# zsc/MOSS-TTSD

Measured on AMD Instinct MI355X. Metric: audio codec tokens/sec/node (decode, bf16, batch 32 @ 4k ctx), higher is better.
Workload: dtype bf16; 1 GPU; configs[2]: batch 32 synthetic dialogues/GPU, 4k-token KV context, top-k/top-p sampling on 8 channels, decode steps at full context; batch_per_gpu=32, context=4096, prompt=512, layers=28, hidden=2048, parallelism=dp1 (batch shard, no per-step collective)

## Files before the change

### include/mtts.h

```cpp
#ifndef MTTS_H
#define MTTS_H

#include <stdint.h>

#ifdef __cplusplus
extern "C" {
#endif

#define MTTS_OK 0
#define MTTS_EINVAL (-1)
#define MTTS_EHIP (-2)
#define MTTS_ENOMEM (-3)
#define MTTS_ESTATE (-4)

#define MTTS_CHANNELS 8

typedef struct MttsConfig {
    int32_t vocab_size;
    int32_t hidden_size;
    int32_t intermediate_size;
    int32_t num_hidden_layers;
    int32_t num_attention_heads;
    int32_t num_key_value_heads;
    int32_t head_dim;
    int32_t channels;
    int32_t speech_vocab_size;
    int32_t speech_pad_token;
    int32_t speech_range_lo;
    int32_t speech_range_hi;
    int32_t eos_token_id;
    int32_t max_position;
    float rms_norm_eps;
    int32_t max_batch;
    int32_t max_seq_len;
    int32_t kv_pool_pages;
    int32_t dtype;
} MttsConfig;
#define MTTS_DTYPE_BF16 0
#define MTTS_DTYPE_F32 1
#define MTTS_DTYPE_F16 2

typedef struct MttsSamplerCfg {
    int32_t do_sample;
    int32_t top_k;
    float top_p;
    float one_minus_top_p;
    float temperature;
    float repetition_penalty;
} MttsSamplerCfg;

typedef struct MttsEngine MttsEngine;

const char* mtts_last_error(void);
int32_t mtts_version(void);

int32_t mtts_engine_create(const MttsConfig* cfg, int32_t device, MttsEngine** out);
int32_t mtts_engine_destroy(MttsEngine* e);

int32_t mtts_bind_weight(MttsEngine* e, const char* name, const void* dev_bf16,
                         int64_t rows, int64_t cols, void* stream);
int32_t mtts_bind_rope(MttsEngine* e, const void* dev_cos_bf16, const void* dev_sin_bf16,
                       int32_t rows, void* stream);
int32_t mtts_weights_ready(MttsEngine* e);

int32_t mtts_generate(MttsEngine* e, const int64_t* host_input_ids, const uint8_t* host_attention_mask,
                      int32_t B, int32_t T, int32_t max_length,
                      const MttsSamplerCfg* sampler, uint64_t seed,
                      int64_t* host_out_ids, int32_t out_capacity, int32_t* out_len,
                      const int64_t* host_forced, int32_t forced_len, int64_t* host_decisions,
                      void* stream);

int32_t mtts_begin(MttsEngine* e, const int64_t* host_input_ids, const uint8_t* host_attention_mask,
                   int32_t B, int32_t T, int32_t max_length,
                   const MttsSamplerCfg* sampler, uint64_t seed, void* stream);
int32_t mtts_step(MttsEngine* e, int32_t n_steps, void* stream);
int32_t mtts_sync_state(MttsEngine* e, int32_t* steps_done, int32_t* all_finished, void* stream);
int32_t mtts_read_generated(MttsEngine* e, int64_t* host_gen, int32_t capacity_steps, int32_t* n_steps);
int32_t mtts_set_output_scores(MttsEngine* e, int32_t on);
int32_t mtts_read_scores(MttsEngine* e, float* host_lp, int32_t capacity_steps, int32_t* n_steps);
int32_t mtts_slot_read_scores(MttsEngine* e, int32_t slot, float* host_rows, int32_t capacity_steps, int32_t* n_steps);
int32_t mtts_score(MttsEngine* e, const int64_t* host_input_ids, const uint8_t* host_attention_mask,
                   const int64_t* host_labels, int32_t B, int32_t T, float* host_logp, void* stream);
int32_t mtts_read_logits(MttsEngine* e, uint16_t* host_logits0, uint16_t* host_logits17, void* stream);
int32_t mtts_read_logits_f32(MttsEngine* e, float* host_logits0, float* host_logits17, void* stream);
int32_t mtts_sched_open(MttsEngine* e, int32_t B, int32_t gen_cap, const MttsSamplerCfg* sampler, void* stream);
int32_t mtts_slot_submit(MttsEngine* e, int32_t slot, const int64_t* host_ids, int32_t T, int32_t max_length, uint64_t seed,
                         void* stream);
int32_t mtts_slot_submit_row(MttsEngine* e, int32_t slot, const int64_t* host_ids, int32_t T, int32_t max_length, uint64_t seed,
                             int32_t row_id, void* stream);
int32_t mtts_set_row_ids(MttsEngine* e, const int32_t* host_row_ids, int32_t n);
int32_t mtts_set_takes(MttsEngine* e, int32_t n);
int32_t mtts_slot_fork(MttsEngine* e, int32_t src_slot, int32_t dst_slot, uint64_t seed, int32_t row_id, void* stream);
int32_t mtts_slot_states(MttsEngine* e, int32_t* host_state, void* stream);
int32_t mtts_slot_read(MttsEngine* e, int32_t slot, int64_t* host_rows, int32_t capacity_steps, int32_t* n_steps);
int32_t mtts_read_seq_state(MttsEngine* e, int32_t* host_nas, int32_t* host_unfinished, int32_t* host_kv_len, void* stream);
int32_t mtts_slot_evict(MttsEngine* e, int32_t slot, void* stream);
int32_t mtts_kv_pool_state(MttsEngine* e, int32_t* total_pages, int32_t* free_pages, int32_t* max_pages_per_seq);
int32_t mtts_read_page_table(MttsEngine* e, int32_t* host_table, int32_t* host_n_pages);
int32_t mtts_set_forced_mode(MttsEngine* e, int32_t as_draw);
int32_t mtts_debug_read_device_page_table(MttsEngine* e, int32_t* host_table, void* stream);
int32_t mtts_export_codes(MttsEngine* e, int32_t first, int32_t n, int64_t* dev_codes, void* stream);
int32_t mtts_profile_enable(MttsEngine* e, int32_t on);
int32_t mtts_profile_read(MttsEngine* e, int32_t which, double* total_ms, int64_t* launches, int64_t* bytes);

int32_t mtts_debug_set_kv_len(MttsEngine* e, int32_t kv_len);
int32_t mtts_debug_kv_pack_stats(MttsEngine* e, int64_t* out6);
int32_t mtts_k_attn_bench(MttsEngine* e, int32_t phase, int32_t iters, float* avg_ms, int64_t* bytes_per_launch);
int32_t mtts_k_gemm_bench(int32_t N, int32_t K, int32_t epi, int32_t ksplit, int32_t waves, int32_t copies,
                          int32_t iters, float* avg_us);

int32_t mtts_k_gemm_bf16(const void* dev_w, const void* dev_x, void* dev_y,
                         int32_t M, int32_t N, int32_t K, int32_t ksplit, void* stream);
int64_t mtts_debug_gemm_depth_launches(void);
int64_t mtts_debug_attn_row_launches(void);
int32_t mtts_k_attn_section(const float* dev_slabs, int32_t ksplit, const void* dev_qnw, const void* dev_knw, const void* dev_cos,
                            const void* dev_sin, float eps, const void* dev_k, const void* dev_v, const int32_t* host_lens,
                            const int32_t* host_page_table, int32_t R, int32_t Lmax, int32_t nq, int32_t nkv, int32_t sealed,
                            int32_t path, void* dev_out, void* dev_kcache, void* dev_vcache, void* dev_kpack, void* dev_vpack,
                            void* stream);
int32_t mtts_k_gemm_swiglu_bf16(const void* dev_w, const void* dev_x, void* dev_y,
                                int32_t M, int32_t N, int32_t K, void* stream);
int32_t mtts_k_rmsnorm(const void* dev_x, const void* dev_w, void* dev_y,
                       int32_t rows, int32_t n, float eps, void* stream);
int32_t mtts_k_rope_kvwrite(const void* dev_qkv, const int32_t* host_pos, const void* dev_qnorm, const void* dev_knorm,
                            const void* dev_cos, const void* dev_sin, int32_t R, int32_t nq, int32_t nkv, float eps,
                            void* dev_q, void* dev_k, void* dev_v, void* stream);
int32_t mtts_k_paged_attn_decode(const void* dev_q, const void* dev_k, const void* dev_v, const int32_t* host_lens,
                                 const int32_t* host_page_table, int32_t R, int32_t Lmax, int32_t nq, int32_t nkv,
                                 void* dev_out, void* stream);
int32_t mtts_k_kv_seal(const void* dev_pages, int32_t npages, void* dev_sealed, int32_t as_k, void* stream);
int32_t mtts_k_head_ce(const void* dev_w, const void* dev_x, const int32_t* host_labels, int32_t M, int32_t N, int32_t K,
                       int32_t n_valid, int32_t segments, float* dev_logp, void* stream);
int32_t mtts_k_sample(const void* dev_logits_bf16, int32_t rows, int32_t vocab,
                      const void* dev_history_bitmap, const MttsSamplerCfg* cfg,
                      int32_t mask_id, uint64_t seed, int32_t step, int32_t channel,
                      int32_t* dev_tokens, void* stream);
int32_t mtts_k_sample_scores(const void* dev_logits_bf16, int32_t rows, int32_t vocab,
                             const void* dev_history_bitmap, const MttsSamplerCfg* cfg,
                             int32_t mask_id, uint64_t seed, int32_t step, int32_t channel,
                             int32_t* dev_tokens, float* dev_logp, void* stream);

typedef struct MttsCodecConfig {
    int32_t nq, codebook_size, rvq_dim, quant_out_dim;
    int32_t adapter_layers, adapter_dim, adapter_heads, adapter_ffn, adapter_max_pos;
    int32_t up_stride;
    int32_t dec_layers, dec_dim, dec_heads, dec_ffn, dec_max_pos, mel_bins;
    int32_t voc_dim, voc_inter, voc_layers, n_fft, hop;
    int32_t mel_n_fft, mel_hop, mel_frames;
    int32_t enc_layers, enc_dim, enc_heads, enc_ffn, enc_max_pos;
    int32_t sem_adapter_layers, pre_rvq_layers, down_pool;
} MttsCodecConfig;

typedef struct MttsCodec MttsCodec;
const char* mtts_codec_last_error(void);
int32_t mtts_codec_create(const MttsCodecConfig* cfg, int32_t device, MttsCodec** out);
int32_t mtts_codec_destroy(MttsCodec* c);
int32_t mtts_codec_bind(MttsCodec* c, const char* role, const float* dev_f32, int64_t n, void* stream);
int32_t mtts_codec_detokenize(MttsCodec* c, const int64_t* dev_codes, const int32_t* host_lens, int32_t B, int32_t T,
                              float* dev_wav, void* stream);
int32_t mtts_codec_detokenize_async(MttsCodec* c, const int64_t* dev_codes, const int32_t* host_lens, int32_t B, int32_t T,
                                    float* dev_wav, void* stream);
int32_t mtts_codec_check(MttsCodec* c, void* stream);
int32_t mtts_codec_tokenize(MttsCodec* c, const float* dev_wav, const int32_t* host_lens, int32_t B, int32_t nsamp,
                            int64_t* dev_codes, int32_t* host_code_lens, void* stream);
int32_t mtts_k_gemm_f32(const float* dev_a, const float* dev_w, const float* dev_bias, float* dev_c,
                        int32_t M, int32_t N, int32_t K, int32_t act, void* stream);
int32_t mtts_k_gemm_planes_bench(int32_t M, int32_t N, int32_t K, int32_t flags, int32_t tile_code, int32_t iters,
                                 float* avg_us, int32_t* code_used);

#ifdef __cplusplus
}
#endif
#endif
```

### moss-ttsd_amd/csrc/attn.hip

```cpp
#include "launch.h"
#include <algorithm>
#include <atomic>
#include <cstdlib>
#ifndef MTTS_PK_WAVES
#define MTTS_PK_WAVES 0
#endif
#if MTTS_PK_WAVES
#define PK_OCC(PK) __attribute__((amdgpu_waves_per_eu((PK) ? MTTS_PK_WAVES : 1, (PK) ? MTTS_PK_WAVES : 8)))
#else
#define PK_OCC(PK)
#endif

__device__ __forceinline__ uint32_t u4c(const u32x4_t& v, int c) { return c == 0 ? v.x : c == 1 ? v.y : c == 2 ? v.z : v.w; }
__device__ __forceinline__ void pk_unit(const u32x4_t* pk, int j, uint32_t w[4]) {
    const uint32_t L0 = u4c(pk[j >> 1], 2 * (j & 1)), L1 = u4c(pk[j >> 1], 2 * (j & 1) + 1);
    const uint32_t N = u4c(pk[8 + (j >> 2)], j & 3);
    const uint32_t lo = pk[12].x, hi = pk[12].y;
    const uint32_t HA = ((N & 0x08080808u) << 4) | __builtin_amdgcn_perm(hi, lo, N & 0x07070707u);
    const uint32_t HB = (N & 0x80808080u) | __builtin_amdgcn_perm(hi, lo, (N >> 4) & 0x07070707u);
    w[0] = __builtin_amdgcn_perm(HA, L0, 0x05010400u);
    w[1] = __builtin_amdgcn_perm(HA, L0, 0x07030602u);
    w[2] = __builtin_amdgcn_perm(HB, L1, 0x05010400u);
    w[3] = __builtin_amdgcn_perm(HB, L1, 0x07030602u);
}

__host__ __device__ constexpr int pk_order(int i) { return i == 0 ? 12 : (i - 1) % 3 == 0 ? 8 + (i - 1) / 3 : 2 * ((i - 1) / 3) + (i - 1) % 3 - 1; }
__device__ bool seal_encode(const u32x4_t (&v)[16], u32x4_t* __restrict__ pk, uint32_t spare, bool unfit) {
    unsigned long long b0 = 0ull, b1 = 0ull;
#pragma unroll
    for (int j = 0; j < 16; ++j)
#pragma unroll
        for (int c = 0; c < 4; ++c)
#pragma unroll
            for (int h = 0; h < 2; ++h) {
                const uint32_t e = (u4c(v[j], c) >> (8 + 16 * h)) & 0x7fu;
                if (e & 64u) b1 |= 1ull << (e & 63u);
                else b0 |= 1ull << e;
            }
    const int n0 = __popcll(b0), n = n0 + __popcll(b1);
    if (n > 8 || unfit) {
        pk[12 * 64] = u32x4_t{0u, 0u, spare, 1u};
        return false;
    }
    unsigned long long dict = 0ull;
    {
        unsigned long long t0 = b0, t1 = b1;
        for (int i = 0; i < n; ++i) {
            uint32_t e;
            if (t0) { e = __ffsll((long long)t0) - 1; t0 &= t0 - 1; }
            else { e = 64 + __ffsll((long long)t1) - 1; t1 &= t1 - 1; }
            dict |= (unsigned long long)e << (8 * i);
        }
    }
    auto code = [&](uint32_t half) -> uint32_t {
        const uint32_t e = (half >> 8) & 0x7fu;
        const uint32_t rank = (e & 64u) ? n0 + __popcll(b1 & ((1ull << (e & 63u)) - 1ull)) : __popcll(b0 & ((1ull << e) - 1ull));
        return ((half >> 12) & 8u) | rank;
    };
    uint32_t lowp[32], nib[16];
#pragma unroll
    for (int j = 0; j < 16; ++j) {
        uint32_t N = 0u;
#pragma unroll
        for (int g = 0; g < 2; ++g) {
            uint32_t L = 0u;
#pragma unroll
            for (int k = 0; k < 4; ++k) {
                const uint32_t half = (u4c(v[j], 2 * g + (k >> 1)) >> (16 * (k & 1))) & 0xffffu;
                L |= (half & 0xffu) << (8 * k);
                N |= code(half) << (8 * k + 4 * g);
            }
            lowp[2 * j + g] = L;
        }
        nib[j] = N;
    }
#pragma unroll
    for (int u = 0; u < 8; ++u) pk[u * 64] = u32x4_t{lowp[4 * u], lowp[4 * u + 1], lowp[4 * u + 2], lowp[4 * u + 3]};
#pragma unroll
    for (int u = 0; u < 4; ++u) pk[(8 + u) * 64] = u32x4_t{nib[4 * u], nib[4 * u + 1], nib[4 * u + 2], nib[4 * u + 3]};
    pk[12 * 64] = u32x4_t{(uint32_t)dict, (uint32_t)(dict >> 32), spare, 0u};
    return true;
}
__device__ bool seal_lane(const u32x4_t* __restrict__ raw, u32x4_t* __restrict__ pk) {
    u32x4_t v[16];
#pragma unroll
    for (int j = 0; j < 16; ++j) v[j] = raw[j * 64];
    return seal_encode(v, pk, 0u, false);
}
__device__ bool seal_lane_k(const u32x4_t* __restrict__ raw, u32x4_t* __restrict__ pk, uint8_t* __restrict__ lds, int lane) {
    u32x4_t v[16];
#pragma unroll
    for (int j = 0; j < 16; ++j) v[j] = raw[j * 64];
    __builtin_amdgcn_wave_barrier();
    uint32_t* row = (uint32_t*)(lds + lane * 128);
#pragma unroll
    for (int j = 0; j < 16; ++j)
#pragma unroll
        for (int c = 0; c < 4; c += 2) {
            const uint32_t a = u4c(v[j], c), b = u4c(v[j], c + 1);
            row[2 * j + (c >> 1)] = ((a >> 7) & 0xffu) | (((a >> 23) & 0xffu) << 8) | (((b >> 7) & 0xffu) << 16) | (((b >> 23) & 0xffu) << 24);
        }
    __builtin_amdgcn_wave_barrier();
    uint32_t a0 = 0u, a1 = 0u, n0 = 0u, n1 = 0u;
    for (int t = 0; t < 64; ++t) {
        const uint32_t e = *(const uint16_t*)(lds + t * 128 + 2 * lane);
        a0 += e & 0xffu; n0 += (e & 0xffu) ? 1u : 0u;
        a1 += e >> 8; n1 += (e >> 8) ? 1u : 0u;
    }
    const int s0 = n0 ? min(max((int)((a0 + n0 / 2) / n0) - 125, -127), 127) : 0;
    const int s1 = n1 ? min(max((int)((a1 + n1 / 2) / n1) - 125, -127), 127) : 0;
    int8_t* sv = (int8_t*)(lds + 8192);
    sv[2 * lane] = (int8_t)s0;
    sv[2 * lane + 1] = (int8_t)s1;
    __builtin_amdgcn_wave_barrier();
    bool unfit = false;
#pragma unroll
    for (int j = 0; j < 16; ++j) {
        uint32_t w[4] = {v[j].x, v[j].y, v[j].z, v[j].w};
#pragma unroll
        for (int c = 0; c < 4; ++c) {
            const uint32_t sh = *(const uint16_t*)(sv + 8 * j + 2 * c);
            uint32_t out = 0u;
#pragma unroll
            for (int h = 0; h < 2; ++h) {
                uint32_t b = (w[c] >> (16 * h)) & 0xffffu;
                const int sft = (int)(int8_t)((sh >> (8 * h)) & 0xffu);
                const int e = (int)((b >> 7) & 0xffu);
                if (e == 0) {
                    if ((b & 0x7fu) && sft) unfit = true;
                } else {
                    const int e2 = e - sft;
                    if (e == 255 ? sft != 0 : (e2 < 1 || e2 > 254)) unfit = true;
                    else b = (b - ((uint32_t)sft << 7)) & 0xffffu;
                }
                out |= b << (16 * h);
            }
            w[c] = out;
        }
        v[j] = u32x4_t{w[0], w[1], w[2], w[3]};
    }
    return seal_encode(v, pk, ((uint32_t)s0 & 0xffu) | (((uint32_t)s1 & 0xffu) << 8), unfit);
}
__device__ bool seal_lane_v(const u32x4_t* __restrict__ raw, u32x4_t* __restrict__ pk, uint8_t* __restrict__ lds, int lane) {
    u32x4_t v[16];
#pragma unroll
    for (int j = 0; j < 16; ++j) v[j] = raw[j * 64];
    const int sub = lane >> 5;
    __builtin_amdgcn_wave_barrier();
    uint32_t* row = (uint32_t*)(lds + lane * 128);
#pragma unroll
    for (int it = 0; it < 16; ++it)
#pragma unroll
        for (int h = 0; h < 2; ++h) {
            uint32_t sum = 0u, cnt = 0u;
#pragma unroll
            for (int c = 0; c < 4; ++c) {
                const uint32_t e = (u4c(v[it], c) >> (7 + 16 * h)) & 0xffu;
                sum += e;
                cnt += e ? 1u : 0u;
            }
            row[2 * it + h] = sum | (cnt << 16);
        }
    __builtin_amdgcn_wave_barrier();
    int mean;
    {
        const int t = lane, st = (t >> 1) & 1, j = 2 * (t >> 2) + (t & 1);
        uint32_t tot = 0u, cn = 0u;
        for (int d = 0; d < 32; ++d) {
            const uint32_t w = ((const uint32_t*)(lds + (st * 32 + d) * 128))[j];
            tot += w & 0xffffu;
            cn += w >> 16;
// ... 1214 lines not shown
```

### moss-ttsd_amd/csrc/engine.h

```cpp
#pragma once
#include <hip/hip_runtime.h>

#include <algorithm>
#include <cstdarg>
#include <cstdio>
#include <cstdlib>
#include <cstring>
#include <memory>
#include <string>
#include <vector>

#include "launch.h"

#define MTTS_LOCAL __attribute__((visibility("hidden")))
extern MTTS_LOCAL thread_local char g_err[512];
MTTS_LOCAL int fail(int code, const char* fmt, ...) __attribute__((format(printf, 2, 3)));
#define HIPCHK(x)                                                                          \
    do {                                                                                   \
        hipError_t _e = (x);                                                               \
        if (_e != hipSuccess) return fail(MTTS_EHIP, "%s: %s (%s:%d)", #x, hipGetErrorString(_e), __FILE__, __LINE__); \
    } while (0)
#define TRY(x)             \
    do {                   \
        int _r = (x);      \
        if (_r) return _r; \
    } while (0)

static inline int round_up(int a, int b) { return (a + b - 1) / b * b; }
static inline hipStream_t S(void* s) { return (hipStream_t)s; }
static inline int gemm_depth_env() {
    const char* g = getenv("MTTS_GEMM_DEPTH");
    return (g && atoi(g) == 0) ? 0 : 1;
}

template <typename T>
static int dalloc(T** p, size_t n, bool zero = true) {
    HIPCHK(hipMalloc((void**)p, n * sizeof(T)));
    if (zero) HIPCHK(hipMemset(*p, 0, n * sizeof(T)));
    return 0;
}

struct DevBufs {
    struct Buf { void* p; bool pinned; };
    std::vector<Buf> bufs;
    std::string free_error;
    DevBufs() = default;
    DevBufs(const DevBufs&) = delete;
    DevBufs& operator=(const DevBufs&) = delete;
    ~DevBufs() { free_all(); }
    template <typename T>
    int get(T** out, size_t n, bool zero = true) {
        TRY(dalloc(out, n, zero));
        bufs.push_back({(void*)*out, false});
        return 0;
    }
    template <typename T>
    int get_pinned(T** out, size_t n) {
        HIPCHK(hipHostMalloc((void**)out, n * sizeof(T)));
        bufs.push_back({(void*)*out, true});
        memset((void*)*out, 0, n * sizeof(T));
        return 0;
    }
    template <typename T>
    void release(T*& p) {
        if (!p) return;
        auto it = std::find_if(bufs.begin(), bufs.end(), [&](const Buf& b) { return b.p == (void*)p; });
        if (it == bufs.end()) note(hipErrorInvalidValue, (void*)p);
        else { free_one(*it); bufs.erase(it); }
        p = nullptr;
    }
    void free_all() {
        for (const Buf& b : bufs) free_one(b);
        bufs.clear();
    }
private:
    void free_one(const Buf& b) {
        const hipError_t r = b.pinned ? hipHostFree(b.p) : hipFree(b.p);
        if (r != hipSuccess) note(r, b.p);
    }
    void note(hipError_t r, void* p) {
        if (!free_error.empty()) return;
        char msg[160];
        snprintf(msg, sizeof(msg), "freeing %p: %s", p, hipGetErrorString(r));
        free_error = msg;
    }
};

static inline int full_cap_for(int vocab) { int p = 1; while (p < vocab) p <<= 1; return vocab > SAMP_CAND ? p : 0; }
static inline int alloc_scratch(DevBufs& m, SampleScratch& sc, int rows, int vocab) {
    const int fc = full_cap_for(vocab);
    TRY(m.get(&sc.overflow, (size_t)rows));
    if (fc) {
        TRY(m.get(&sc.full_val, (size_t)rows * fc, false));
        TRY(m.get(&sc.full_idx, (size_t)rows * fc, false));
        TRY(m.get(&sc.nuc_cnt, (size_t)rows * 2048));
        TRY(m.get(&sc.nuc_mass, (size_t)rows * 2048));
    }
    TRY(m.get(&sc.hist, (size_t)rows * 2048));
    TRY(m.get(&sc.slice_val, (size_t)rows * SAMP_NS));
    TRY(m.get(&sc.slice_idx, (size_t)rows * SAMP_NS));
    TRY(m.get(&sc.cand_val, (size_t)rows * SAMP_CAND));
    TRY(m.get(&sc.cand_idx, (size_t)rows * SAMP_CAND));
    TRY(m.get(&sc.cand_n, (size_t)rows));
    return 0;
}
static inline int alloc_lp_scratch(DevBufs& m, SampleScratch& sc, int rows) {
    if (sc.lp) return 0;
    TRY(m.get(&sc.slice_sum, (size_t)rows * SAMP_NS));
    TRY(m.get(&sc.lp, (size_t)rows * 8));
    return 0;
}

struct Layer {
    void *wqkv = nullptr, *wo = nullptr, *wgu = nullptr, *wd = nullptr;
    void *ln_in = nullptr, *ln_post = nullptr, *qn = nullptr, *kn = nullptr;
    int bound = 0;
};

enum { PROF_SCORES = 0, PROF_PV = 1, PROF_GEMM = 2, PROF_STEP = 3,
       PROF_CE = 4,
       PROF_N = 5 };

struct MttsEngine {
    DevBufs mem;
    MttsConfig cfg;
    int device = 0;
    int H, I, L, nq, nkv, V0, Vs, Vs_pad, V0_pad, qkv_rows;
    std::vector<Layer> layers;
    void* emb[8] = {nullptr};
    void* head0 = nullptr;
    void* heads17 = nullptr;
    void* final_norm = nullptr;
    uint16_t *rope_cos = nullptr, *rope_sin = nullptr;
    int rope_rows = 0;
    int emb_bound = 0, norm_bound = 0;
    const uint16_t** d_tables = nullptr;
    GemmPlan p_qkv, p_o, p_gu, p_d, p_h0, p_h17;
    float* partial = nullptr;
    float* partial2 = nullptr;
    void *x2 = nullptr, *act_rm = nullptr;
    int small_rows = SMALL_RP;
    int gemm_depth = 1;
    void *x = nullptr, *xn = nullptr, *attn_p = nullptr, *act_p = nullptr, *qbuf = nullptr, *hlast = nullptr, *xh = nullptr;
    void *logits0 = nullptr, *logits17 = nullptr, *join_logits0 = nullptr, *join_logits17 = nullptr;
    void* scores = nullptr;
    float *stats = nullptr, *opart = nullptr;
    void *kcache = nullptr, *vcache = nullptr;
    size_t layer_stride = 0;
    int total_pages = 0, max_pages = 0, nchunks_max = 0;
    int32_t* d_page_table = nullptr;
    std::vector<int32_t> h_page_table;
    std::vector<int32_t> free_pages;
    std::vector<int32_t> n_pages;
    std::vector<int32_t> page_owners;
    std::vector<char> slot_live;
    PageEdits pending_edits;
    int forced_draw = 0;
    std::vector<int32_t> next_row_ids;
    int next_takes = 1;
    int takes = 1;
    bool f32 = false;
    int h16 = 0;
    struct LayerF32 { float *wqkv = nullptr, *wo = nullptr, *wgu = nullptr, *wd = nullptr, *ln_in = nullptr, *ln_post = nullptr, *qn = nullptr, *kn = nullptr; };
    std::vector<LayerF32> lf;
    float* embf[8] = {nullptr};
    const float** d_tables_f = nullptr;
    float *final_norm_f = nullptr, *rope_cos_f = nullptr, *rope_sin_f = nullptr;
    float *kcache_f = nullptr, *vcache_f = nullptr;
    float *xf = nullptr, *xnf = nullptr, *qkvf = nullptr, *qbuf_f = nullptr, *attnf = nullptr, *yf = nullptr, *guf = nullptr,
          *actf = nullptr, *hlast_f = nullptr, *scores_f = nullptr;
    SeqState* d_seqs = nullptr;
    RowMeta* d_meta = nullptr;
    LoopState* d_ls = nullptr;
    LoopState* h_ls = nullptr;
    SeqState* h_seqs = nullptr;
    int32_t *d_decisions = nullptr, *d_cur = nullptr, *d_gen = nullptr, *d_declog = nullptr, *d_forced = nullptr,
            *d_tf = nullptr;
    uint32_t* d_bitmaps = nullptr;
    int bm_words = 0;
    MttsSamplerCfg* d_scfg = nullptr;
    SampleScratch sscr;
    int ch0_sampled = 0;
    float* d_lp = nullptr;
    int lp_cap = 0;
    int scores_next = 0;
    int scores_on = 0;
    bool run_open = false;
    int32_t* d_sc_labels = nullptr;
    float* d_sc_logp = nullptr;
    size_t sc_cap_rows = 0;
    float* sc_part = nullptr;
    float* sc_logits = nullptr;
    int32_t* d_pf_tokens = nullptr;
    RowMeta* d_pf_meta = nullptr;
    size_t pf_cap_rows = 0;
    int gen_cap = 0;
    int B = 0, T = 0, base_length = 0, max_length = 0, max_steps = 0, steps_issued = 0;
    bool continuous = false;
    std::vector<int> join_step;
    std::vector<int> n_real;
    int max_real = 0;
    uint64_t seed = 0;
    bool began = false, has_forced = false;
    struct StepGraph { int B, pages, forced, ch0, scores, row; hipGraphExec_t exec; };
    std::vector<StepGraph> graphs;
    hipStream_t cap_stream = nullptr;
    bool use_graphs = true;
    int kv_pack = 1;
    void *kpack = nullptr, *vpack = nullptr;
    size_t pk_layer_stride = 0;
    unsigned long long *d_seal_cnt = nullptr, *h_seal_cnt = nullptr;
    std::vector<char> pack_k_on, pack_v_on;
    int pack_min_work = 512;
    int fuse_qkv_max = 2560;
    int attn_row = 1;
    int n_cus = 0;
    int pf_mfma_pages = 0;
    bool prof = false;
    std::vector<std::pair<hipEvent_t, hipEvent_t>> ev[PROF_N];
    int64_t prof_bytes[PROF_N] = {0, 0, 0, 0, 0};
};

static inline bool attn_row_auto(int rows, int nkv, int pages_bound, int n_cus) {
    (void)pages_bound;
    return n_cus > 0 && rows * nkv >= n_cus;
}
static inline bool attn_row_shape(const MttsEngine* e, int pages_bound) {
    if (e->attn_row == 0 || e->f32) return false;
    return e->attn_row == 2 || attn_row_auto(e->B, e->nkv, pages_bound, e->n_cus);
}

static inline KvPack layer_pack(MttsEngine* e, int n, int pages_bound) {
    KvPack pk{nullptr, nullptr};
    if (e->B * pages_bound < e->pack_min_work) return pk;
    if (e->kpack && e->pack_k_on[n]) pk.k = (uint8_t*)e->kpack + e->pk_layer_stride * n;
    if (e->vpack && e->pack_v_on[n]) pk.v = (uint8_t*)e->vpack + e->pk_layer_stride * n;
    return pk;
}
```

### moss-ttsd_amd/csrc/engine.hip

```cpp
#include "engine.h"

#define FLUSH_STEPS 7
#define LINGER_STEPS 14
static inline int linger_bound(int B) { return 6 * B + 8; }

thread_local char g_err[512] = "";
int fail(int code, const char* fmt, ...) {
    va_list ap;
    va_start(ap, fmt);
    vsnprintf(g_err, sizeof(g_err), fmt, ap);
    va_end(ap);
    return code;
}

const char* mtts_last_error(void) { return g_err; }
int32_t mtts_version(void) { return 202; }

static void pool_reset(MttsEngine* e) {
    e->free_pages.resize(e->total_pages);
    for (int i = 0; i < e->total_pages; ++i) e->free_pages[i] = e->total_pages - 1 - i;
    if (const char* g = getenv("MTTS_PAGE_SHUFFLE")) {
        uint64_t x = 0x9E3779B97F4A7C15ull ^ (uint64_t)atoll(g);
        for (int i = e->total_pages - 1; i > 0; --i) {
            x = x * 6364136223846793005ull + 1442695040888963407ull;
// ... 35 lines not shown
}
static int pool_share(MttsEngine* e, int src, int dst, int npages, hipStream_t st) {
    for (int i = 0; i < npages; ++i) {
        const int page = e->h_page_table[(size_t)src * e->max_pages + i];
        e->page_owners[page]++;
        TRY(pool_append(e, dst, page, st));
    }
    return 0;
}
static void pool_release(MttsEngine* e, int b) {
    for (int i = e->n_pages[b] - 1; i >= 0; --i) {
        const int page = e->h_page_table[(size_t)b * e->max_pages + i];
        if (--e->page_owners[page] == 0) e->free_pages.push_back(page);
    }
    e->n_pages[b] = 0;
    int k = 0;
    for (int i = 0; i < e->pending_edits.n; ++i)
        if (e->pending_edits.idx[i] / e->max_pages != b) {
            e->pending_edits.idx[k] = e->pending_edits.idx[i];
            e->pending_edits.val[k++] = e->pending_edits.val[i];
        }
    e->pending_edits.n = k;
}

static int create_f32(MttsEngine* e) {
    const size_t H = e->H, I = e->I, D = MTTS_HD;
    e->lf.resize(e->L);
    for (auto& l : e->lf) {
        TRY(e->mem.get(&l.wqkv, (size_t)e->qkv_rows * H, false));
        TRY(e->mem.get(&l.wo, H * e->nq * D, false));
        TRY(e->mem.get(&l.wgu, 2 * I * H, false));
        TRY(e->mem.get(&l.wd, H * I, false));
        TRY(e->mem.get(&l.ln_in, H)); TRY(e->mem.get(&l.ln_post, H)); TRY(e->mem.get(&l.qn, D)); TRY(e->mem.get(&l.kn, D));
    }
    TRY(e->mem.get(&e->embf[0], (size_t)e->V0 * H, false));
    for (int ch = 1; ch < 8; ++ch) TRY(e->mem.get(&e->embf[ch], (size_t)e->Vs * H, false));
    TRY(e->mem.get(&e->final_norm_f, H));
    TRY(e->mem.get(&e->d_tables_f, 8));
    HIPCHK(hipMemcpy((void*)e->d_tables_f, e->embf, 8 * sizeof(void*), hipMemcpyHostToDevice));
    const size_t P = MTTS_PF32CAP;
    TRY(e->mem.get(&e->xf, P * H)); TRY(e->mem.get(&e->xnf, P * H)); TRY(e->mem.get(&e->yf, P * H));
    TRY(e->mem.get(&e->qkvf, P * e->qkv_rows)); TRY(e->mem.get(&e->qbuf_f, P * e->nq * D)); TRY(e->mem.get(&e->attnf, P * e->nq * D));
    TRY(e->mem.get(&e->guf, P * 2 * I)); TRY(e->mem.get(&e->actf, P * I));
    TRY(e->mem.get(&e->hlast_f, (size_t)MTTS_RCAP * H));
    TRY(e->mem.get((float**)&e->logits0, (size_t)MTTS_RCAP * e->V0_pad));
    TRY(e->mem.get((float**)&e->logits17, (size_t)MTTS_RCAP * 7 * e->Vs_pad));
    return 0;
}

static int forward_rows_f32(MttsEngine* e, const int32_t* d_tokens, const RowMeta* d_meta, int R, int heads, hipStream_t st) {
    const int H = e->H, I = e->I, nq = e->nq, nkv = e->nkv;
    const float eps = e->cfg.rms_norm_eps, scale = 1.0f / sqrtf((float)MTTS_HD);
    const int Lmax = e->max_pages * MTTS_PAGE, h16 = e->h16;
    const bool dec = heads == 1;
    launch_f32_embed_norm(d_tokens, d_meta, e->d_tables_f, e->lf[0].ln_in, e->xf, e->xnf, R, H, eps, h16, st);
    for (int n = 0; n < e->L; ++n) {
        auto& l = e->lf[n];
        float* kc = e->kcache_f + e->layer_stride * n;
        float* vc = e->vcache_f + e->layer_stride * n;
        launch_f32_linear(l.wqkv, e->xnf, e->qkvf, R, e->qkv_rows, H, e->qkv_rows, h16, dec, st);
        launch_f32_qkv_post(e->qkvf, e->qkv_rows, d_meta, l.qn, l.kn, e->rope_cos_f, e->rope_sin_f, e->qbuf_f, kc, vc,
                            e->d_page_table, e->max_pages, e->total_pages, R, nq, nkv, eps, h16, st);
        launch_f32_attn(e->qbuf_f, kc, vc, e->d_page_table, d_meta, e->scores_f, e->attnf, R, e->max_pages, e->total_pages, nq,
                        nkv, scale, Lmax, h16, st);
        launch_f32_linear(l.wo, e->attnf, e->yf, R, H, nq * MTTS_HD, H, h16, dec, st);
        launch_f32_resid_norm(e->yf, e->xf, l.ln_post, e->xnf, nullptr, d_meta, R, H, eps, h16, st);
        launch_f32_linear(l.wgu, e->xnf, e->guf, R, 2 * I, H, 2 * I, h16, dec, st);
        launch_f32_swiglu(e->guf, e->actf, R, I, h16, st);
        launch_f32_linear(l.wd, e->actf, e->yf, R, H, I, H, h16, dec, st);
        const bool lastl = n == e->L - 1;
        launch_f32_resid_norm(e->yf, e->xf, lastl ? e->final_norm_f : e->lf[n + 1].ln_in, e->xnf, lastl ? e->hlast_f : nullptr,
                              d_meta, R, H, eps, h16, st);
    }
    if (heads) {
        const float* xin = heads == 1 ? e->xnf : e->hlast_f;
        launch_f32_linear(e->embf[0], xin, (float*)e->logits0, e->B, e->V0, H, e->V0_pad, h16, true, st);
        for (int c = 1; c < 8; ++c)
            launch_f32_linear(e->embf[c], xin, (float*)e->logits17 + (size_t)(c - 1) * e->Vs_pad, e->B, e->Vs, H, 7 * e->Vs_pad, h16, true, st);
    }
    HIPCHK(hipGetLastError());
    return MTTS_OK;
}

static void drop_graphs(MttsEngine* e) {
    for (auto& g : e->graphs) hipGraphExecDestroy(g.exec);
    e->graphs.clear();
}

int32_t mtts_engine_create(const MttsConfig* c, int32_t device, MttsEngine** out) {
    if (!c || !out) return fail(MTTS_EINVAL, "null argument");
    if (c->head_dim != MTTS_HD) return fail(MTTS_EINVAL, "head_dim must be 128 (got %d)", c->head_dim);
    if (c->channels != 8) return fail(MTTS_EINVAL, "channels must be 8");
    if (c->hidden_size % 16 || c->intermediate_size % 16) return fail(MTTS_EINVAL, "hidden/intermediate must be multiples of 16");
    if (c->hidden_size > 8192) return fail(MTTS_EINVAL, "hidden_size > 8192 not built (resid_norm keeps a row in registers)");
    if (c->num_attention_heads % c->num_key_value_heads) return fail(MTTS_EINVAL, "bad GQA ratio");
    int G = c->num_attention_heads / c->num_key_value_heads;
    if (G != 1 && G != 2 && G != 4) return fail(MTTS_EINVAL, "GQA group %d not built (1,2,4)", G);
    if (c->max_batch < 1 || c->max_batch > MTTS_RCAP) return fail(MTTS_EINVAL, "max_batch must be 1..128");
    if (c->vocab_size <= 152694 || c->speech_vocab_size <= 1024)
        return fail(MTTS_EINVAL, "vocab too small for the reference's hard-coded mask ids 152694 / 1024");
    if (c->dtype != MTTS_DTYPE_BF16 && c->dtype != MTTS_DTYPE_F32 && c->dtype != MTTS_DTYPE_F16)
        return fail(MTTS_EINVAL, "dtype %d not built (bf16 = 0, fp32 = 1, fp16 = 2)", c->dtype);
    if (c->kv_pool_pages < 0) return fail(MTTS_EINVAL, "kv_pool_pages must be >= 0");
    HIPCHK(hipSetDevice(device));
    struct Destroy {
        void operator()(MttsEngine* p) const {
            const std::string keep = g_err;
            mtts_engine_destroy(p);
            snprintf(g_err, sizeof(g_err), "%s", keep.c_str());
        }
    };
    std::unique_ptr<MttsEngine, Destroy> holder(new MttsEngine());
    MttsEngine* e = holder.get();
    DevBufs& m = e->mem;
    e->cfg = *c;
    e->device = device;
    if (const char* g = getenv("MTTS_GRAPHS")) e->use_graphs = atoi(g) != 0;
    if (const char* g = getenv("MTTS_FUSE_QKV_MAX")) e->fuse_qkv_max = atoi(g);
    if (const char* g = getenv("MTTS_KV_PACK")) e->kv_pack = atoi(g);
    if (const char* g = getenv("MTTS_KV_PACK_MIN")) e->pack_min_work = atoi(g);
    if (const char* g = getenv("MTTS_PREFILL_MFMA_PAGES")) e->pf_mfma_pages = atoi(g);
    if (const char* g = getenv("MTTS_ATTN_ROW")) e->attn_row = std::min(std::max(atoi(g), 0), 2);
    HIPCHK(hipDeviceGetAttribute(&e->n_cus, hipDeviceAttributeMultiprocessorCount, device));
    if (e->attn_row && attn_row_prepare()) {
        if (e->attn_row == 2) return fail(MTTS_EINVAL, "attn_row_kernel: the dynamic LDS limit could not be raised");
        e->attn_row = 0;
    }
    if (const char* g = getenv("MTTS_SMALL_ROWS")) e->small_rows = std::min(std::max(atoi(g), 0), SMALL_RP);
    e->gemm_depth = gemm_depth_env();
    e->H = c->hidden_size; e->I = c->intermediate_size; e->L = c->num_hidden_layers;
    e->nq = c->num_attention_heads; e->nkv = c->num_key_value_heads;
    e->V0 = c->vocab_size; e->Vs = c->speech_vocab_size;
    e->V0_pad = round_up(e->V0, 32); e->Vs_pad = round_up(e->Vs, 32);
    e->qkv_rows = (e->nq + 2 * e->nkv) * MTTS_HD;
    e->layers.resize(e->L);
    const int H = e->H, I = e->I;
    e->f32 = c->dtype != MTTS_DTYPE_BF16;
    e->h16 = c->dtype == MTTS_DTYPE_F16;
    if (e->f32) TRY(create_f32(e));
    if (!e->f32) {
        for (auto& l : e->layers) {
            TRY(m.get((uint16_t**)&l.wqkv, (size_t)e->qkv_rows * H));
            TRY(m.get((uint16_t**)&l.wo, (size_t)H * e->nq * MTTS_HD));
            TRY(m.get((uint16_t**)&l.wgu, (size_t)2 * I * H));
            TRY(m.get((uint16_t**)&l.wd, (size_t)round_up(H, 32) * I));
            TRY(m.get((uint16_t**)&l.ln_in, (size_t)H));
            TRY(m.get((uint16_t**)&l.ln_post, (size_t)H));
            TRY(m.get((uint16_t**)&l.qn, (size_t)MTTS_HD));
            TRY(m.get((uint16_t**)&l.kn, (size_t)MTTS_HD));
        }
        TRY(m.get((uint16_t**)&e->emb[0], (size_t)e->V0 * H, false));
        for (int ch = 1; ch < 8; ++ch) TRY(m.get((uint16_t**)&e->emb[ch], (size_t)e->Vs * H, false));
        TRY(m.get((uint16_t**)&e->head0, (size_t)e->V0_pad * H));
        TRY(m.get((uint16_t**)&e->heads17, (size_t)7 * e->Vs_pad * H));
        TRY(m.get((uint16_t**)&e->final_norm, (size_t)H));
        TRY(m.get(&e->d_tables, 8));
        HIPCHK(hipMemcpy((void*)e->d_tables, e->emb, 8 * sizeof(void*), hipMemcpyHostToDevice));
    }
    e->p_qkv = mtts_plan_gemm(e->qkv_rows, H, 0);
    e->p_o = mtts_plan_gemm(round_up(H, 32), e->nq * MTTS_HD, 0);
    e->p_gu = mtts_plan_gemm(2 * I, H, 1);
    e->p_d = mtts_plan_gemm(round_up(H, 32), I, 0);
    e->p_h0 = mtts_plan_gemm(e->V0_pad, H, 1);
    e->p_h17 = mtts_plan_gemm(7 * e->Vs_pad, H, 1);
    for (GemmPlan* p : {&e->p_qkv, &e->p_o, &e->p_gu, &e->p_d, &e->p_h0, &e->p_h17}) p->depth = e->gemm_depth;
    size_t pmax = (size_t)8 * std::max(e->qkv_rows, round_up(H, 32));
    if (!e->f32) {
        TRY(m.get(&e->partial, pmax * MTTS_PFCAP));
        TRY(m.get(&e->partial2, (size_t)8 * round_up(H, 32) * MTTS_PFCAP));
        TRY(m.get((uint16_t**)&e->x2, (size_t)MTTS_MAXR * H));
        TRY(m.get((uint16_t**)&e->act_rm, (size_t)MTTS_MAXR * I));
        TRY(m.get((uint16_t**)&e->x, (size_t)MTTS_PFCAP * H));
        TRY(m.get((uint16_t**)&e->xn, (size_t)MTTS_PFCAP * H));
        TRY(m.get((uint16_t**)&e->xh, (size_t)MTTS_RCAP * H));
        TRY(m.get((uint16_t**)&e->hlast, (size_t)MTTS_RCAP * H));
        TRY(m.get((uint16_t**)&e->attn_p, (size_t)MTTS_PFCAP * e->nq * MTTS_HD));
        TRY(m.get((uint16_t**)&e->act_p, (size_t)MTTS_PFCAP * I));
        TRY(m.get((uint16_t**)&e->qbuf, (size_t)MTTS_PFCAP * e->nq * MTTS_HD));
        TRY(m.get((uint16_t**)&e->logits0, (size_t)MTTS_RCAP * e->V0_pad));
        TRY(m.get((uint16_t**)&e->logits17, (size_t)MTTS_RCAP * 7 * e->Vs_pad));
        TRY(m.get((uint16_t**)&e->join_logits0, (size_t)MTTS_MAXR * e->V0_pad));
        TRY(m.get((uint16_t**)&e->join_logits17, (size_t)MTTS_MAXR * 7 * e->Vs_pad));
    }
    e->max_pages = (c->max_seq_len + MTTS_PAGE - 1) / MTTS_PAGE + 1;
    e->total_pages = c->kv_pool_pages > 0 ? c->kv_pool_pages : e->max_pages * c->max_batch;
    e->nchunks_max = (e->max_pages + ATT_PB - 1) / ATT_PB;
    e->layer_stride = (size_t)e->total_pages * e->nkv * MTTS_PAGE * MTTS_HD;
    if (e->f32) {
        TRY(m.get(&e->kcache_f, e->layer_stride * e->L));
        TRY(m.get(&e->vcache_f, e->layer_stride * e->L));
        TRY(m.get(&e->scores_f, (size_t)MTTS_PF32CAP * e->nq * e->max_pages * MTTS_PAGE, false));
    } else {
        TRY(m.get((uint16_t**)&e->kcache, e->layer_stride * e->L));
        TRY(m.get((uint16_t**)&e->vcache, e->layer_stride * e->L));
        if (e->kv_pack) {
            e->pk_layer_stride = (size_t)e->total_pages * e->nkv * MTTS_PKU * 64 * 16;
            size_t free_b = 0, total_b = 0;
            const size_t need = 2 * e->pk_layer_stride * e->L;
            if (hipMemGetInfo(&free_b, &total_b) != hipSuccess || need + ((size_t)8 << 30) > free_b) {
                fprintf(stderr, "mtts: sealed KV pages off: %.1f GB needed, %.1f GB free (8 GB kept for the run)\n", need / 1e9, free_b / 1e9);
                e->kv_pack = 0;
            }
        }
        if (e->kv_pack) {
            TRY(m.get((uint8_t**)&e->kpack, e->pk_layer_stride * e->L));
            TRY(m.get((uint8_t**)&e->vpack, e->pk_layer_stride * e->L));
            TRY(m.get(&e->d_seal_cnt, (size_t)e->L * 4));
            TRY(m.get_pinned(&e->h_seal_cnt, (size_t)e->L * 4));
            e->pack_k_on.assign(e->L, 1);
            e->pack_v_on.assign(e->L, 1);
        }
    }
// ... 26 lines not shown

int32_t mtts_engine_destroy(MttsEngine* e) {
    if (!e) return MTTS_OK;
    hipSetDevice(e->device);
    hipDeviceSynchronize();
    drop_graphs(e);
    if (e->cap_stream) hipStreamDestroy(e->cap_stream);
    for (int w = 0; w < PROF_N; ++w) for (auto& pr : e->ev[w]) { hipEventDestroy(pr.first); hipEventDestroy(pr.second); }
    e->mem.free_all();
    const std::string err = e->mem.free_error;
    delete e;
    return err.empty() ? MTTS_OK : fail(MTTS_EHIP, "mtts_engine_destroy: %s", err.c_str());
}

struct WeightSlot {
    int64_t rows = 0, cols = 0;
    void* copy_to = nullptr;
    void* pack_to = nullptr;
    int rows_pad = 0, row_mul = 1, row_off = 0;
    float* f32_to = nullptr;
    int64_t f32_row = 0;
    int* bound = nullptr;
    int bit = 0;
};

static int resolve_weight(MttsEngine* e, const char* name_c, WeightSlot& w) {
    const std::string name(name_c);
    const int64_t H = e->H, I = e->I, D = MTTS_HD, Hp = round_up(e->H, 32), QD = e->nq * D, KD = e->nkv * D;
    int ch = -1;
    if (sscanf(name_c, "model.embedding_list.%d.weight", &ch) == 1 && name.size() > 7 && name.compare(name.size() - 7, 7, ".weight") == 0) {
        if (ch < 0 || ch > 7) return fail(MTTS_EINVAL, "bad channel in %s", name_c);
        w.rows = ch == 0 ? e->V0 : e->Vs; w.cols = H;
        w.copy_to = e->emb[ch]; w.f32_to = e->embf[ch];
        w.pack_to = ch == 0 ? e->head0 : e->heads17;
        w.rows_pad = ch == 0 ? e->V0_pad : 7 * e->Vs_pad;
        w.row_off = ch == 0 ? 0 : (ch - 1) * e->Vs_pad;
        w.bound = &e->emb_bound; w.bit = 1 << ch;
        return MTTS_OK;
    }
    if (name == "model.language_model.norm.weight") {
        w.rows = H; w.cols = 1; w.copy_to = e->final_norm; w.f32_to = e->final_norm_f; w.bound = &e->norm_bound; w.bit = 1;
        return MTTS_OK;
    }
    if (name.find("lm_heads.") == 0 || name == "model.language_model.embed_tokens.weight") return MTTS_OK;
    int n = -1;
    char rest[128];
    if (sscanf(name_c, "model.language_model.layers.%d.%127s", &n, rest) != 2) return fail(MTTS_EINVAL, "unknown tensor %s", name_c);
    if (n < 0 || n >= e->L) return fail(MTTS_EINVAL, "layer index out of range in %s", name_c);
    Layer& l = e->layers[n];
    const MttsEngine::LayerF32 f = e->f32 ? e->lf[n] : MttsEngine::LayerF32{};
    const struct { const char* name; int64_t rows, cols; void* bf; float* f32; int rows_pad, row_mul, row_off; int64_t f32_row; } t[] = {
        {"input_layernorm.weight", H, 1, l.ln_in, f.ln_in, 0, 1, 0, 0},
        {"post_attention_layernorm.weight", H, 1, l.ln_post, f.ln_post, 0, 1, 0, 0},
        {"self_attn.q_norm.weight", D, 1, l.qn, f.qn, 0, 1, 0, 0},
        {"self_attn.k_norm.weight", D, 1, l.kn, f.kn, 0, 1, 0, 0},
        {"self_attn.q_proj.weight", QD, H, l.wqkv, f.wqkv, e->qkv_rows, 1, 0, 0},
        {"self_attn.k_proj.weight", KD, H, l.wqkv, f.wqkv, e->qkv_rows, 1, (int)QD, QD},
        {"self_attn.v_proj.weight", KD, H, l.wqkv, f.wqkv, e->qkv_rows, 1, (int)(QD + KD), QD + KD},
        {"self_attn.o_proj.weight", H, QD, l.wo, f.wo, (int)Hp, 1, 0, 0},
        {"mlp.gate_proj.weight", I, H, l.wgu, f.wgu, (int)(2 * I), 2, 0, 0},
        {"mlp.up_proj.weight", I, H, l.wgu, f.wgu, (int)(2 * I), 2, 1, I},
        {"mlp.down_proj.weight", H, I, l.wd, f.wd, (int)Hp, 1, 0, 0},
    };
    for (int i = 0; i < 11; ++i)
        if (!strcmp(rest, t[i].name)) {
            w.rows = t[i].rows; w.cols = t[i].cols;
            (t[i].cols == 1 ? w.copy_to : w.pack_to) = t[i].bf;
            w.rows_pad = t[i].rows_pad; w.row_mul = t[i].row_mul; w.row_off = t[i].row_off;
            w.f32_to = t[i].f32; w.f32_row = t[i].f32_row;
            w.bound = &l.bound; w.bit = 1 << i;
            return MTTS_OK;
        }
    return fail(MTTS_EINVAL, "unknown tensor %s", name_c);
}

int32_t mtts_bind_weight(MttsEngine* e, const char* name_c, const void* src, int64_t rows, int64_t cols, void* stream) {
    if (!e || !name_c || !src) return fail(MTTS_EINVAL, "null argument");
    HIPCHK(hipSetDevice(e->device));
    drop_graphs(e);
    hipStream_t st = S(stream);
    WeightSlot w;
    TRY(resolve_weight(e, name_c, w));
    if (!w.bound) return MTTS_OK;
    const bool shape_ok = w.cols == 1 ? (rows == w.rows && cols == 1) || (rows == 1 && cols == w.rows) : rows == w.rows && cols == w.cols;
    if (!shape_ok)
        return fail(MTTS_EINVAL, "%s: expected [%lld,%lld] got [%lld,%lld]", name_c, (long long)w.rows, (long long)w.cols, (long long)rows, (long long)cols);
    const size_t n = (size_t)w.rows * w.cols;
    if (e->f32) {
        HIPCHK(hipMemcpyAsync(w.f32_to + w.f32_row * w.cols, src, n * 4, hipMemcpyDeviceToDevice, st));
    } else {
        if (w.copy_to) HIPCHK(hipMemcpyAsync(w.copy_to, src, n * 2, hipMemcpyDeviceToDevice, st));
        if (w.pack_to) launch_pack_weight(src, w.pack_to, (int)w.rows, (int)w.cols, w.rows_pad, w.row_mul, w.row_off, st);
        HIPCHK(hipGetLastError());
    }
    *w.bound |= w.bit;
    return MTTS_OK;
}

template <typename T>
static int bind_rope_tables(MttsEngine* e, T*& c, T*& s, const void* cosb, const void* sinb, int rows, hipStream_t st) {
    e->mem.release(c);
    e->mem.release(s);
    TRY(e->mem.get(&c, (size_t)rows * 64, false));
    TRY(e->mem.get(&s, (size_t)rows * 64, false));
    HIPCHK(hipMemcpyAsync(c, cosb, (size_t)rows * 64 * sizeof(T), hipMemcpyDeviceToDevice, st));
    HIPCHK(hipMemcpyAsync(s, sinb, (size_t)rows * 64 * sizeof(T), hipMemcpyDeviceToDevice, st));
    e->rope_rows = rows;
    return MTTS_OK;
}
int32_t mtts_bind_rope(MttsEngine* e, const void* cosb, const void* sinb, int32_t rows, void* stream) {
    if (!e || !cosb || !sinb || rows < 1) return fail(MTTS_EINVAL, "bad rope table");
    HIPCHK(hipSetDevice(e->device));
    drop_graphs(e);
    if (e->f32) return bind_rope_tables(e, e->rope_cos_f, e->rope_sin_f, cosb, sinb, rows, S(stream));
    return bind_rope_tables(e, e->rope_cos, e->rope_sin, cosb, sinb, rows, S(stream));
}

int32_t mtts_weights_ready(MttsEngine* e) {
    if (!e) return fail(MTTS_EINVAL, "null engine");
    if (e->emb_bound != 0xff) return fail(MTTS_ESTATE, "embedding tables missing (mask %x)", e->emb_bound);
    if (!e->norm_bound) return fail(MTTS_ESTATE, "final norm missing");
    if (!e->rope_rows) return fail(MTTS_ESTATE, "rope table missing");
    for (int n = 0; n < e->L; ++n)
        if (e->layers[n].bound != 2047) return fail(MTTS_ESTATE, "layer %d incomplete (mask %x)", n, e->layers[n].bound);
    return MTTS_OK;
}

static void prof_begin(MttsEngine* e, int which, hipStream_t st, hipEvent_t* a) {
    if (!e->prof) return;
    hipEvent_t s0, s1;
    hipEventCreate(&s0); hipEventCreate(&s1);
    hipEventRecord(s0, st);
    e->ev[which].push_back({s0, s1});
    *a = s1;
}
static void prof_end(MttsEngine* e, hipStream_t st, hipEvent_t a) {
    if (!e->prof) return;
    hipEventRecord(a, st);
}

static int pack_policy_reset(MttsEngine* e, hipStream_t st) {
    if (!e->d_seal_cnt) return 0;
    HIPCHK(hipMemsetAsync(e->d_seal_cnt, 0, (size_t)e->L * 4 * sizeof(unsigned long long), st));
    bool changed = false;
    for (int n = 0; n < e->L; ++n) { changed |= !e->pack_k_on[n] || !e->pack_v_on[n]; e->pack_k_on[n] = 1; e->pack_v_on[n] = 1; }
    if (changed) drop_graphs(e);
    return 0;
}
static int attend_layer(MttsEngine* e, int n, const RowMeta* d_meta, int R, int pages_bound, int ks_qkv, int nphases, bool prefill,
                        bool fused, bool sealed, hipStream_t st, int64_t kv_tokens_hint) {
    static const AttnPhase decode_ph[3] = {ATTN_SCORES, ATTN_PV, ATTN_COMBINE}, prefill_ph[3] = {ATTN_PF_SCORES, ATTN_PF_PV, ATTN_PF_COMBINE};
    Layer& l = e->layers[n];
    const float eps = e->cfg.rms_norm_eps, scale = 1.0f / sqrtf((float)MTTS_HD);
    uint16_t* kc = (uint16_t*)e->kcache + e->layer_stride * n;
    uint16_t* vc = (uint16_t*)e->vcache + e->layer_stride * n;
    const QkvFuse fz{e->partial, ks_qkv, e->qkv_rows, (const uint16_t*)l.qn, (const uint16_t*)l.kn, e->rope_cos, e->rope_sin, eps};
    const KvPack pk = layer_pack(e, n, pages_bound);
    const KvPack* pkp = (sealed && (pk.k || pk.v)) ? &pk : nullptr;
    if (!prefill && sealed && nphases == 3 && attn_row_shape(e, pages_bound) && attn_row_fits(e->nq / e->nkv, &fz, pkp, pages_bound)) {
        hipEvent_t ev = nullptr;
        prof_begin(e, PROF_SCORES, st, &ev);
        if (const int rc = launch_attn(e->qbuf, kc, vc, e->d_page_table, d_meta, e->scores, e->stats, e->opart, e->attn_p, R, pages_bound,
                                       e->max_pages, e->total_pages, e->nchunks_max, e->nq, e->nkv, scale, &fz, ATTN_ROW, st, pkp))
            return fail(MTTS_EINVAL, rc == -2 ? "the whole-row attention kernel does not take this launch" : "attention group size not built");
        prof_end(e, st, ev);
        if (e->prof) e->prof_bytes[PROF_SCORES] += 2 * kv_tokens_hint * e->nkv * MTTS_HD * 2;
        return 0;
    }
    if (!fused)
        launch_qkv_post(e->partial, ks_qkv, e->qkv_rows, d_meta, l.qn, l.kn, e->rope_cos, e->rope_sin, e->qbuf,
                        kc, vc, e->d_page_table, e->max_pages, e->total_pages, R, e->nq, e->nkv, eps, st);
    for (int i = 0; i < nphases; ++i) {
        hipEvent_t ev = nullptr;
        if (i < 2) prof_begin(e, i == 0 ? PROF_SCORES : PROF_PV, st, &ev);
        if (launch_attn(e->qbuf, kc, vc, e->d_page_table, d_meta, e->scores, e->stats, e->opart, e->attn_p, R,
                        pages_bound, e->max_pages, e->total_pages, e->nchunks_max, e->nq, e->nkv, scale,
                        fused ? &fz : nullptr, (prefill ? prefill_ph : decode_ph)[i], st, pkp))
            return fail(MTTS_EINVAL, "attention group size not built");
        if (i < 2) prof_end(e, st, ev);
    }
    if (e->prof) {
        e->prof_bytes[PROF_SCORES] += kv_tokens_hint * e->nkv * MTTS_HD * 2;
        e->prof_bytes[PROF_PV] += kv_tokens_hint * e->nkv * MTTS_HD * 2;
    }
    return 0;
}
static bool small_path_fits(MttsEngine* e) {
    const int H = e->H;
    if (H > 8192 || H % 8 || e->I % 8) return false;
    const int lim = 64 * 1024 - 33 * 1024;
    return mtts_small_lds_bytes(e->p_qkv, H, PRO_NORM) <= lim && mtts_small_lds_bytes(e->p_d, e->I, PRO_ROWS) <= lim &&
           mtts_small_lds_bytes(e->p_o, e->nq * MTTS_HD, PRO_COMBINE) <= lim;
}
static int forward_small(MttsEngine* e, const RowMeta* d_meta, int pages_bound, hipStream_t st, int64_t kv_tokens_hint) {
    const int H = e->H, I = e->I, nq = e->nq, nkv = e->nkv, Hp = round_up(H, 32), R = MTTS_MAXR;
    const float eps = e->cfg.rms_norm_eps;
    uint16_t* xa = (uint16_t*)e->x;
    uint16_t* xb = (uint16_t*)e->x2;
    SmallPro base{};
    base.rows = e->B; base.eps = eps; base.slab_npad = Hp;
    for (int n = 0; n < e->L; ++n) {
        Layer& l = e->layers[n];
        SmallPro pq = base;
        pq.x_in = xa; pq.x_out = xb; pq.slabs = e->partial2; pq.ksplit = n ? e->p_d.ksplit : 0; pq.norm_w = (const uint16_t*)l.ln_in;
        launch_gemv_small(EPI_PARTIAL, PRO_NORM, e->p_qkv, l.wqkv, H, e->qkv_rows, e->qkv_rows, e->partial, nullptr, pq, st);
        TRY(attend_layer(e, n, d_meta, R, pages_bound, e->p_qkv.ksplit, 2, false, e->B * pages_bound <= e->fuse_qkv_max, true, st,
                         kv_tokens_hint));
        SmallPro po = base;
        po.opart = e->opart; po.meta = d_meta; po.nchunks_max = e->nchunks_max; po.nq = nq; po.pages_per_chunk = ATT_PB;
        launch_gemv_small(EPI_PARTIAL, PRO_COMBINE, e->p_o, l.wo, nq * MTTS_HD, Hp, Hp, e->partial2, nullptr, po, st);
        SmallPro pg = base;
        pg.x_in = xb; pg.x_out = xa; pg.slabs = e->partial2; pg.ksplit = e->p_o.ksplit; pg.norm_w = (const uint16_t*)l.ln_post;
        launch_gemv_small(EPI_SILU_RM, PRO_NORM, e->p_gu, l.wgu, H, 2 * I, 2 * I, nullptr, (uint16_t*)e->act_rm, pg, st);
        SmallPro pd = base;
        pd.xrows = (const uint16_t*)e->act_rm;
        launch_gemv_small(EPI_PARTIAL, PRO_ROWS, e->p_d, l.wd, I, Hp, Hp, e->partial2, nullptr, pd, st);
    }
    if (e->kpack)
        launch_kv_seal_rows(e->kcache, e->vcache, e->kpack, e->vpack, e->d_page_table, d_meta, R, e->max_pages, e->total_pages, nkv, e->L, e->d_seal_cnt, st);
    SmallPro ph = base;
    ph.x_in = xa; ph.x_out = nullptr; ph.slabs = e->partial2; ph.ksplit = e->p_d.ksplit; ph.norm_w = (const uint16_t*)e->final_norm;
    launch_gemv_small(EPI_BF16, PRO_NORM, e->p_h0, e->head0, H, e->V0_pad, e->V0, nullptr, (uint16_t*)e->logits0, ph, st);
    launch_gemv_small(EPI_BF16, PRO_NORM, e->p_h17, e->heads17, H, 7 * e->Vs_pad, 7 * e->Vs_pad, nullptr, (uint16_t*)e->logits17, ph, st);
    HIPCHK(hipGetLastError());
    return MTTS_OK;
}

static int forward_rows(MttsEngine* e, const int32_t* d_tokens, const RowMeta* d_meta, int R, int pages_bound,
                        int heads, hipStream_t st, int64_t kv_tokens_hint) {
    const int H = e->H, I = e->I, nq = e->nq, nkv = e->nkv;
    const float eps = e->cfg.rms_norm_eps;
    const int Hp = round_up(H, 32);
    const int mb = (R + 31) / 32;
    const bool tiled = heads != 1;
    if (e->f32) return forward_rows_f32(e, d_tokens, d_meta, heads == 1 ? e->B : R, heads, st);
    launch_embed_norm(d_tokens, d_meta, e->d_tables, e->layers[0].ln_in, e->x, e->xn, R, H, eps, st);
    if (heads == 1 && e->B <= e->small_rows && small_path_fits(e)) return forward_small(e, d_meta, pages_bound, st, kv_tokens_hint);
    for (int n = 0; n < e->L; ++n) {
        Layer& l = e->layers[n];
        const int ks_qkv = tiled ? mtts_tile_ksplit(e->qkv_rows, H, 1024) : e->p_qkv.ksplit;
        const int ks_o = tiled ? mtts_tile_ksplit(Hp, nq * MTTS_HD, 1024) : e->p_o.ksplit;
        const int ks_d = tiled ? mtts_tile_ksplit(Hp, I, 1024) : e->p_d.ksplit;
        if (tiled) launch_gemm_tile(EPI_PARTIAL, R, ks_qkv, l.wqkv, e->xn, H, e->qkv_rows, e->qkv_rows, e->partial, nullptr, st);
        else launch_gemm(EPI_PARTIAL, mb, e->p_qkv, l.wqkv, e->xn, H, e->qkv_rows, e->qkv_rows, e->partial, nullptr, st);
        TRY(attend_layer(e, n, d_meta, R, pages_bound, ks_qkv, 3, heads != 1 && pages_bound >= e->pf_mfma_pages,
                         heads == 1 && e->B * pages_bound <= e->fuse_qkv_max, heads == 1, st, kv_tokens_hint));
        if (tiled) launch_gemm_tile(EPI_PARTIAL, R, ks_o, l.wo, e->attn_p, nq * MTTS_HD, Hp, Hp, e->partial, nullptr, st);
        else launch_gemm(EPI_PARTIAL, mb, e->p_o, l.wo, e->attn_p, nq * MTTS_HD, Hp, Hp, e->partial, nullptr, st);
        launch_resid_norm(e->partial, ks_o, Hp, e->x, l.ln_post, e->xn, nullptr, d_meta, R, H, eps, st);
        if (tiled) {
            launch_gemm_tile(EPI_SILU, R, 1, l.wgu, e->xn, H, 2 * I, 2 * I, nullptr, (uint16_t*)e->act_p, st);
            launch_gemm_tile(EPI_PARTIAL, R, ks_d, l.wd, e->act_p, I, Hp, Hp, e->partial, nullptr, st);
        } else {
            launch_gemm(EPI_SILU, mb, e->p_gu, l.wgu, e->xn, H, 2 * I, 2 * I, nullptr, (uint16_t*)e->act_p, st);
            launch_gemm(EPI_PARTIAL, mb, e->p_d, l.wd, e->act_p, I, Hp, Hp, e->partial, nullptr, st);
        }
        const bool lastl = (n == e->L - 1);
        const void* nw = lastl ? e->final_norm : e->layers[n + 1].ln_in;
        launch_resid_norm(e->partial, ks_d, Hp, e->x, nw, e->xn, lastl ? e->hlast : nullptr, d_meta, R, H, eps, st);
    }
    if (e->kpack)
        launch_kv_seal_rows(e->kcache, e->vcache, e->kpack, e->vpack, e->d_page_table, d_meta, R, e->max_pages, e->total_pages, nkv, e->L, e->d_seal_cnt, st);
    if (heads) {
        const void* xin = e->xn;
        int hmb = mb;
        if (heads == 2) {
            hmb = (e->B + 31) / 32;
            launch_pack_rows(e->hlast, e->xh, e->B, H, hmb, st);
            xin = e->xh;
        }
        launch_gemm(EPI_BF16, hmb, e->p_h0, e->head0, xin, H, e->V0_pad, e->V0, nullptr, (uint16_t*)e->logits0, st);
        launch_gemm(EPI_BF16, hmb, e->p_h17, e->heads17, xin, H, 7 * e->Vs_pad, 7 * e->Vs_pad, nullptr, (uint16_t*)e->logits17, st);
    }
    HIPCHK(hipGetLastError());
    return MTTS_OK;
}

static int prefill_staged(MttsEngine* e, size_t Mpad, int pages_bound, int last_heads, hipStream_t st) {
    const size_t pfcap = e->f32 ? MTTS_PF32CAP : MTTS_PFCAP;
    for (size_t off = 0; off < Mpad; off += pfcap) {
        const int rows = (int)std::min<size_t>(pfcap, Mpad - off);
        TRY(forward_rows(e, e->d_pf_tokens + off * 8, e->d_pf_meta + off, rows, pages_bound, off + rows >= Mpad ? last_heads : 0, st, 0));
    }
    return 0;
}

static int ensure_gen_storage(MttsEngine* e, int steps) {
    if (steps <= e->gen_cap) return 0;
    e->mem.release(e->d_gen); e->mem.release(e->d_declog); e->mem.release(e->d_forced);
    drop_graphs(e);
    e->gen_cap = steps;
    const size_t n = (size_t)e->cfg.max_batch * steps * 8;
    TRY(e->mem.get(&e->d_gen, n));
    TRY(e->mem.get(&e->d_declog, n));
    TRY(e->mem.get(&e->d_forced, n, false));
    return 0;
}

static int start_scores(MttsEngine* e, hipStream_t st) {
    e->scores_on = e->scores_next;
    if (!e->scores_on) return 0;
    if (!e->sscr.lp) {
        drop_graphs(e);
        TRY(alloc_lp_scratch(e->mem, e->sscr, e->cfg.max_batch));
    }
    const size_t n = (size_t)e->cfg.max_batch * e->gen_cap * 8;
    if (!e->d_lp || e->lp_cap != e->gen_cap) {
        e->mem.release(e->d_lp);
        drop_graphs(e);
        TRY(e->mem.get(&e->d_lp, n, false));
        e->lp_cap = e->gen_cap;
    }
    HIPCHK(hipMemsetAsync(e->d_lp, 0xff, n * sizeof(float), st));
    return 0;
}

static int grow_prefill_staging(MttsEngine* e, size_t rows) {
    if (rows <= e->pf_cap_rows) return 0;
    e->mem.release(e->d_pf_tokens); e->mem.release(e->d_pf_meta);
    e->pf_cap_rows = 0;
    TRY(e->mem.get(&e->d_pf_tokens, rows * 8, false));
    TRY(e->mem.get(&e->d_pf_meta, rows, false));
    e->pf_cap_rows = rows;
    return 0;
}

static const SeqState IDLE_SEQ{-1, 0, 0, 0, 0, 0, 0, 0, 0};
static int reset_run_state(MttsEngine* e, const std::vector<SeqState>& seqs, bool continuous, const MttsSamplerCfg* sampler, hipStream_t st) {
    HIPCHK(hipMemcpyAsync(e->d_seqs, seqs.data(), seqs.size() * sizeof(SeqState), hipMemcpyHostToDevice, st));
    if (continuous) e->forced_draw = 0;
    LoopState ls{0, 0, continuous ? 1 : 0, e->B, 0, e->gen_cap, e->forced_draw, e->f32 ? 1 : 0};
    e->continuous = continuous;
    e->join_step.assign(MTTS_RCAP, 0);
    HIPCHK(hipMemcpyAsync(e->d_ls, &ls, sizeof(ls), hipMemcpyHostToDevice, st));
    *e->h_ls = ls;
    std::vector<RowMeta> dm(MTTS_RCAP, RowMeta{-1, 0, 0, 0});
    HIPCHK(hipMemcpyAsync(e->d_meta, dm.data(), dm.size() * sizeof(RowMeta), hipMemcpyHostToDevice, st));
    HIPCHK(hipMemcpyAsync(e->d_scfg, sampler, 8 * sizeof(MttsSamplerCfg), hipMemcpyHostToDevice, st));
    e->ch0_sampled = sampler[0].do_sample ? 1 : 0;
    HIPCHK(hipMemsetAsync(e->sscr.hist, 0, (size_t)e->cfg.max_batch * 2048 * 4, st));
    HIPCHK(hipMemsetAsync(e->sscr.cand_n, 0, (size_t)e->cfg.max_batch * 4, st));
    HIPCHK(hipMemsetAsync(e->sscr.overflow, 0, (size_t)e->cfg.max_batch * 4, st));
    HIPCHK(hipStreamSynchronize(st));
    return 0;
}

static int launch_fork_job(MttsEngine* e, ForkJob& job, bool state_rows, hipStream_t st) {
    const int ew = e->f32 ? 4 : 2;
    job.narr = 0;
    auto arr = [&](void* base, size_t stride, size_t bytes) {
        job.base[job.narr] = (uint8_t*)base; job.stride[job.narr] = (int64_t)stride; job.bytes[job.narr++] = (int64_t)bytes;
    };
    arr(e->logits0, (size_t)e->V0_pad * ew, (size_t)e->V0_pad * ew);
    arr(e->logits17, (size_t)7 * e->Vs_pad * ew, (size_t)7 * e->Vs_pad * ew);
    if (state_rows) {
// ... 71 lines not shown
    e->max_steps = max_steps;
    TRY(ensure_gen_storage(e, max_steps));
    TRY(start_scores(e, st));
    size_t Mtot = 0;
    for (int b = 0; b < B; ++b) Mtot += (size_t)round_up(e->n_real[b * takes], MTTS_MAXR);
    size_t Mpad = (Mtot + MTTS_RCAP - 1) / MTTS_RCAP * MTTS_RCAP;
    std::vector<int32_t> toks(Mpad * 8, 0);
    std::vector<RowMeta> metas(Mpad, RowMeta{-1, 0, 0, 0});
    size_t r = 0;
    for (int b = 0; b < B; r = (r + MTTS_MAXR - 1) / MTTS_MAXR * MTTS_MAXR, ++b)
        for (int i = 0; i < e->n_real[b * takes]; ++i, ++r) {
            const int64_t* src = ids + ((size_t)b * T + pad[b] + i) * 8;
            for (int c = 0; c < 8; ++c) {
                int64_t t = src[c];
                int64_t V = c == 0 ? e->V0 : e->Vs;
                if (t < 0 || t >= V) return fail(MTTS_EINVAL, "token %lld out of range on channel %d", (long long)t, c);
                toks[r * 8 + c] = (int32_t)t;
            }
            metas[r] = RowMeta{b * takes, i, i == e->n_real[b * takes] - 1 ? 1 : 0, 0};
        }
    TRY(grow_prefill_staging(e, Mpad));
    HIPCHK(hipMemcpyAsync(e->d_pf_tokens, toks.data(), Mpad * 8 * 4, hipMemcpyHostToDevice, st));
    HIPCHK(hipMemcpyAsync(e->d_pf_meta, metas.data(), Mpad * sizeof(RowMeta), hipMemcpyHostToDevice, st));
    {
        std::vector<uint32_t> bm((size_t)MTTS_RCAP * 8 * e->bm_words, 0u);
        for (int rw = 0; rw < R; ++rw)
            for (int t = 0, b = rw / takes; t < base; ++t)
                for (int c = 0; c < 8; ++c) {
                    int64_t tk = ids[((size_t)b * T + t) * 8 + c];
                    if (tk >= 0 && tk < (int64_t)e->bm_words * 32) bm[((size_t)rw * 8 + c) * e->bm_words + (tk >> 5)] |= 1u << (tk & 31);
                }
        HIPCHK(hipMemcpyAsync(e->d_bitmaps, bm.data(), bm.size() * 4, hipMemcpyHostToDevice, st));
        std::vector<int32_t> tf((size_t)MTTS_RCAP * 7 * 8, 0);
        for (int rw = 0; rw < R; ++rw)
            for (int s = 0, b = rw / takes; s < 7; ++s)
                for (int c = 0; c < 8; ++c) {
                    int64_t tk = ids[((size_t)b * T + base + s) * 8 + c];
                    if (tk < 0 || tk >= (c == 0 ? e->V0 : e->Vs)) return fail(MTTS_EINVAL, "token %lld out of range on channel %d (delayed tail)", (long long)tk, c);
                    tf[((size_t)rw * 7 + s) * 8 + c] = (int32_t)tk;
                }
        HIPCHK(hipMemcpyAsync(e->d_tf, tf.data(), tf.size() * 4, hipMemcpyHostToDevice, st));
        std::vector<SeqState> ss(MTTS_RCAP, IDLE_SEQ);
        if (!e->next_row_ids.empty() && (int)e->next_row_ids.size() != R)
            return fail(MTTS_EINVAL, "mtts_set_row_ids gave %d ids, the batch has %d rows", (int)e->next_row_ids.size(), R);
        for (int b = 0; b < R; ++b)
            ss[b] = SeqState{-1, 1, e->n_real[b], 0, base, max_length, e->next_row_ids.empty() ? b : e->next_row_ids[b], 1, seed};
        e->next_row_ids.clear();
        TRY(reset_run_state(e, ss, false, sampler, st));
    }
    TRY(prefill_staged(e, Mpad, (e->max_real + MTTS_PAGE - 1) / MTTS_PAGE, 2, st));
    if (fork.nr) TRY(launch_fork_job(e, fork, false, st));
    e->began = true;
    e->run_open = true;
    return MTTS_OK;
}

int32_t mtts_set_takes(MttsEngine* e, int32_t n) {
    if (!e) return fail(MTTS_EINVAL, "null engine");
    if (n < 1 || n > MTTS_RCAP) return fail(MTTS_EINVAL, "takes must be 1..%d (got %d)", MTTS_RCAP, n);
    e->next_takes = n;
    return MTTS_OK;
}

int32_t mtts_begin(MttsEngine* e, const int64_t* ids, const uint8_t* mask, int32_t B, int32_t T, int32_t max_length,
                   const MttsSamplerCfg* sampler, uint64_t seed, void* stream) {
    if (!e) return fail(MTTS_EINVAL, "null argument");
    const int takes = e->next_takes;
    e->next_takes = 1;
    return begin_run(e, ids, mask, B, T, max_length, sampler, seed, takes, stream);
}

static int step_body(MttsEngine* e, int pages_bound, hipStream_t st, int64_t kvtok) {
    launch_sample(e->logits0, e->logits17, e->V0, e->Vs, e->Vs_pad, e->d_bitmaps, e->bm_words, e->d_scfg, e->d_ls,
                  e->d_seqs, e->seed, e->d_decisions, &e->d_ls->error, e->B, e->sscr, e->ch0_sampled,
                  full_cap_for(e->V0), e->scores_on, st);
    launch_update(e->d_decisions, e->d_declog, e->has_forced ? e->d_forced : nullptr, e->d_tf, e->d_gen, e->d_cur,
                  e->d_seqs, e->d_meta, e->d_bitmaps, e->bm_words, e->d_ls, e->cfg.eos_token_id,
                  e->cfg.speech_pad_token, e->cfg.speech_range_lo, e->cfg.speech_range_hi,
                  e->scores_on ? e->sscr.lp : nullptr, e->scores_on ? e->d_lp : nullptr, st);
    return forward_rows(e, e->d_cur, e->d_meta, round_up(e->B, 32), pages_bound, 1, st, kvtok);
}

static int step_graph(MttsEngine* e, int pages, hipGraphExec_t* out) {
    const int forced = e->has_forced ? 1 : 0, row = attn_row_shape(e, pages) ? 1 : 0;
    for (auto& g : e->graphs)
        if (g.B == e->B && g.pages == pages && g.forced == forced && g.ch0 == e->ch0_sampled && g.scores == e->scores_on && g.row == row) {
            *out = g.exec;
            return MTTS_OK;
        }
    if (e->graphs.size() >= 256) drop_graphs(e);
    if (!e->cap_stream) HIPCHK(hipStreamCreateWithFlags(&e->cap_stream, hipStreamNonBlocking));
    hipGraph_t g = nullptr;
    HIPCHK(hipStreamBeginCapture(e->cap_stream, hipStreamCaptureModeRelaxed));
    int rc = step_body(e, pages, e->cap_stream, 0);
    hipError_t ce = hipStreamEndCapture(e->cap_stream, &g);
    if (rc) { if (g) hipGraphDestroy(g); return rc; }
    HIPCHK(ce);
    hipGraphExec_t exec = nullptr;
    hipError_t ie = hipGraphInstantiate(&exec, g, nullptr, nullptr, 0);
    hipGraphDestroy(g);
    HIPCHK(ie);
    e->graphs.push_back({e->B, pages, forced, e->ch0_sampled, e->scores_on, row, exec});
    *out = exec;
    return MTTS_OK;
}

static int issue_steps(MttsEngine* e, int n, hipStream_t st) {
    for (int i = 0; i < n; ++i) {
        if (e->steps_issued >= e->max_steps) break;
        int len_bound = 1;
        for (int b = 0; b < e->B; ++b) {
            if (!e->slot_live[b]) continue;
            const int len = e->n_real[b] + e->steps_issued + 1;
            len_bound = std::max(len_bound, len);
            TRY(pool_grow(e, b, (len + MTTS_PAGE - 1) / MTTS_PAGE, st));
        }
        TRY(pool_flush(e, st));
        const int pages_bound = (len_bound + MTTS_PAGE - 1) / MTTS_PAGE;
        if (e->use_graphs && !e->prof) {
            hipGraphExec_t exec = nullptr;
            TRY(step_graph(e, std::min(round_up(pages_bound, ATT_PB), e->max_pages), &exec));
            HIPCHK(hipGraphLaunch(exec, st));
        } else {
            hipEvent_t ev = nullptr;
            prof_begin(e, PROF_STEP, st, &ev);
            int64_t kvtok = 0;
            for (int b = 0; b < e->B; ++b) if (e->slot_live[b]) kvtok += e->n_real[b] + e->steps_issued + 1;
            TRY(step_body(e, pages_bound, st, kvtok));
            prof_end(e, st, ev);
        }
        e->steps_issued++;
    }
    return MTTS_OK;
}

int32_t mtts_step(MttsEngine* e, int32_t n_steps, void* stream) {
    if (!e || !e->began) return fail(MTTS_ESTATE, "mtts_begin has not run");
    HIPCHK(hipSetDevice(e->device));
    return issue_steps(e, n_steps, S(stream));
}

int32_t mtts_sync_state(MttsEngine* e, int32_t* steps_done, int32_t* all_finished, void* stream) {
    if (!e || !e->began) return fail(MTTS_ESTATE, "mtts_begin has not run");
    HIPCHK(hipSetDevice(e->device));
    HIPCHK(hipMemcpyAsync(e->h_ls, e->d_ls, sizeof(LoopState), hipMemcpyDeviceToHost, S(stream)));
    if (!e->continuous) HIPCHK(hipMemcpyAsync(e->h_seqs, e->d_seqs, e->B * sizeof(SeqState), hipMemcpyDeviceToHost, S(stream)));
    if (e->d_seal_cnt) HIPCHK(hipMemcpyAsync(e->h_seal_cnt, e->d_seal_cnt, (size_t)e->L * 4 * sizeof(unsigned long long), hipMemcpyDeviceToHost, S(stream)));
    HIPCHK(hipStreamSynchronize(S(stream)));
    if (e->d_seal_cnt && e->kv_pack == 1) {
        bool changed = false;
        for (int n = 0; n < e->L; ++n) {
            const unsigned long long* c = e->h_seal_cnt + (size_t)n * 4;
            const bool k_on = c[0] + c[1] < 16 || c[1] * 8 <= c[0] + c[1], v_on = c[2] + c[3] < 16 || c[3] * 8 <= c[2] + c[3];
            changed |= (k_on != (bool)e->pack_k_on[n]) || (v_on != (bool)e->pack_v_on[n]);
            e->pack_k_on[n] = k_on; e->pack_v_on[n] = v_on;
        }
        if (changed) drop_graphs(e);
    }
    if (e->h_ls->error) return fail(MTTS_EINVAL, "device sampler error %d: more than 4096 candidate tokens (set top_k so that the k-th score's radix bin holds <= 4096 tokens)", e->h_ls->error);
    if (!e->continuous) {
        const SeqState* ss = e->h_seqs;
        for (int b = 0; b < e->B; ++b)
            if (e->slot_live[b] && ss[b].step > 0 && !ss[b].unfinished && ss[b].active != 2) { e->slot_live[b] = 0; pool_release(e, b); }
    }
    if (steps_done) *steps_done = e->h_ls->step;
    if (all_finished) *all_finished = e->h_ls->done;
    if (e->h_ls->done && !e->continuous) e->run_open = false;
    return MTTS_OK;
}

template <typename Src, typename Dst>
static int read_slots(MttsEngine* e, const Src* d_src, int slot0, int nslots, int steps, Dst* host) {
    std::vector<Src> tmp((size_t)std::max(steps, 1) * 8);
    for (int b = 0; b < nslots; ++b) {
        if (steps) HIPCHK(hipMemcpy(tmp.data(), d_src + (size_t)(slot0 + b) * e->gen_cap * 8, (size_t)steps * 8 * sizeof(Src), hipMemcpyDeviceToHost));
        for (int s = 0; s < steps; ++s)
            for (int c = 0; c < 8; ++c) host[((size_t)s * nslots + b) * 8 + c] = tmp[(size_t)s * 8 + c];
    }
    return MTTS_OK;
}
template <typename Src, typename Dst>
static int read_rows(MttsEngine* e, const Src* d_src, Dst* host, int capacity_steps, int* n_steps) {
    const int steps = e->h_ls->step;
    if (steps > capacity_steps) return fail(MTTS_EINVAL, "output buffer holds %d steps, need %d", capacity_steps, steps);
    TRY(read_slots(e, d_src, 0, e->B, steps, host));
// ... 555 lines not shown
```

### moss-ttsd_amd/csrc/gemm.hip

```cpp
#include "launch.h"


template <int WAVES, int EPI, int MB>
__global__ __launch_bounds__(WAVES * 64) void gemm_skinny_kernel(
    const u32x4_t* __restrict__ Wp, const u32x4_t* __restrict__ Xp, int KT, int kt_per_split,
    int kt_per_wave, float* __restrict__ partial, uint16_t* __restrict__ out, int Npad, int n_valid) {
    __shared__ float red[WAVES][16][64];
    const int nt = blockIdx.x, ks = blockIdx.y;
    const int wave = threadIdx.x >> 6, lane = threadIdx.x & 63;
    int kt0 = ks * kt_per_split + wave * kt_per_wave;
    int kt1 = min(min(kt0 + kt_per_wave, (ks + 1) * kt_per_split), KT);
    f32x16_t acc[MB];
#pragma unroll
    for (int mb = 0; mb < MB; ++mb)
#pragma unroll
        for (int i = 0; i < 16; ++i) acc[mb][i] = 0.f;
    const u32x4_t* wp = Wp + ((size_t)nt * KT + kt0) * 64 + lane;
    const u32x4_t* xp = Xp + (size_t)kt0 * 64 + lane;
    const size_t xtile = (size_t)KT * 64;
    constexpr int U = (MB == 1) ? 8 : 4;
    int n = kt1 - kt0;
    int i = 0;
    for (; i + U <= n; i += U) {
        u32x4_t a[U], b[U][MB];
#pragma unroll
        for (int u = 0; u < U; ++u) a[u] = __builtin_nontemporal_load(wp + (size_t)(i + u) * 64);
#pragma unroll
        for (int u = 0; u < U; ++u)
#pragma unroll
            for (int mb = 0; mb < MB; ++mb) b[u][mb] = xp[(size_t)(i + u) * 64 + mb * xtile];
#pragma unroll
        for (int u = 0; u < U; ++u)
#pragma unroll
            for (int mb = 0; mb < MB; ++mb)
                acc[mb] = __builtin_amdgcn_mfma_f32_32x32x16_bf16(*(bf16x8_t*)&a[u], *(bf16x8_t*)&b[u][mb], acc[mb], 0, 0, 0);
    }
    for (; i < n; ++i) {
        u32x4_t a = __builtin_nontemporal_load(wp + (size_t)i * 64);
#pragma unroll
        for (int mb = 0; mb < MB; ++mb) {
            u32x4_t b = xp[(size_t)i * 64 + mb * xtile];
            acc[mb] = __builtin_amdgcn_mfma_f32_32x32x16_bf16(*(bf16x8_t*)&a, *(bf16x8_t*)&b, acc[mb], 0, 0, 0);
        }
    }
    const int l2 = threadIdx.x & 63;
#pragma unroll
    for (int mb = 0; mb < MB; ++mb) {
        if (mb) __syncthreads();
#pragma unroll
        for (int r = 0; r < 16; ++r) red[wave][r][lane] = acc[mb][r];
        __syncthreads();
        for (int q = threadIdx.x >> 6; q < 4; q += WAVES) {
            float v[4];
#pragma unroll
            for (int j = 0; j < 4; ++j) {
                float s = red[0][4 * q + j][l2];
#pragma unroll
                for (int w = 1; w < WAVES; ++w) s += red[w][4 * q + j][l2];
                v[j] = s;
            }
            const int row = mb * 32 + (l2 & 31);
            const int nl = 8 * q + 4 * (l2 >> 5);
            const int n0 = nt * 32 + nl;
            if (EPI == EPI_PARTIAL) {
                float4 o = make_float4(v[0], v[1], v[2], v[3]);
                *(float4*)(partial + ((size_t)ks * MTTS_PFCAP + row) * Npad + n0) = o;
            } else if (EPI == EPI_BF16) {
                uint16_t* o = out + (size_t)row * Npad + n0;
                if (n0 + 3 < n_valid) *(u32x2_t*)o = u32x2_t{pack2(v[0], v[1]), pack2(v[2], v[3])};
                else {
#pragma unroll
                    for (int j = 0; j < 4; ++j)
                        if (n0 + j < n_valid) o[j] = f2bf(v[j]);
                }
            } else {
#pragma unroll
                for (int j = 0; j < 2; ++j) {
                    float g = rbf(v[2 * j]), u = rbf(v[2 * j + 1]);
                    float a = rbf(g / (1.0f + expf(-g)));
                    int idx = (n0 >> 1) + j;
                    out[xpack_off(row, idx, Npad >> 1)] = f2bf(a * u);
                }
            }
// ... 31 lines not shown
    __shared__ float red[WAVES][16][64];
    const int nt = blockIdx.x, ks = blockIdx.y;
    const int wave = threadIdx.x >> 6, lane = threadIdx.x & 63;
    const int kt0 = (ks * WAVES + wave) * KTW;
    const u32x4_t* wp = Wp + ((size_t)nt * KT + kt0) * 64 + lane;
    const u32x4_t* xp = Xp + (size_t)kt0 * 64 + lane;
    u32x4_t a[KTW], b[KTW];
#pragma unroll
    for (int u = 0; u < KTW; ++u) b[u] = xp[(size_t)u * 64];
    __builtin_amdgcn_sched_barrier(0);
#pragma unroll
    for (int u = 0; u < KTW; ++u) {
        a[u] = __builtin_nontemporal_load(wp + (size_t)u * 64);
        __builtin_amdgcn_sched_barrier(0);
    }
    f32x16_t acc;
#pragma unroll
    for (int i = 0; i < 16; ++i) acc[i] = 0.f;
#pragma unroll
    for (int u = 0; u < KTW; ++u)
        acc = __builtin_amdgcn_mfma_f32_32x32x16_bf16(*(bf16x8_t*)&a[u], *(bf16x8_t*)&b[u], acc, 0, 0, 0);
#pragma unroll
    for (int r = 0; r < 16; ++r) red[wave][r][lane] = acc[r];
    __syncthreads();
    for (int q = wave; q < 4; q += WAVES) {
        float v[4];
#pragma unroll
        for (int j = 0; j < 4; ++j) {
            float s = red[0][4 * q + j][lane];
#pragma unroll
            for (int w = 1; w < WAVES; ++w) s += red[w][4 * q + j][lane];
            v[j] = s;
        }
        skinny_store<EPI>(v, lane & 31, nt * 32 + 8 * q + 4 * (lane >> 5), ks, partial, out, Npad, n_valid);
    }
}

template <int WAVES, int KTW>
__global__ __launch_bounds__(WAVES * 64) void gemm_gateup48_kernel(
    const u32x4_t* __restrict__ Wp, const u32x4_t* __restrict__ Xp, int KT, uint16_t* __restrict__ out, int Npad) {
    __shared__ float red[WAVES][24][64];
    const int p = blockIdx.x >> 1, o = blockIdx.x & 1;
    const int tf = 3 * p + 2 * o, th = 3 * p + 1;
    const int wave = threadIdx.x >> 6, lane = threadIdx.x & 63;
    const int kt0 = wave * KTW;
    const int hl = (((lane >> 4) & 1) == o) ? lane : (lane ^ 16);
    const u32x4_t* wp = Wp + ((size_t)tf * KT + kt0) * 64 + lane;
    const u32x4_t* hp = Wp + ((size_t)th * KT + kt0) * 64 + hl;
    const u32x4_t* xp = Xp + (size_t)kt0 * 64 + lane;
    u32x4_t a[KTW], h[KTW], b[KTW];
#pragma unroll
    for (int u = 0; u < KTW; ++u) b[u] = xp[(size_t)u * 64];
    __builtin_amdgcn_sched_barrier(0);
#pragma unroll
    for (int u = 0; u < KTW; ++u) {
        a[u] = __builtin_nontemporal_load(wp + (size_t)u * 64);
        h[u] = __builtin_nontemporal_load(hp + (size_t)u * 64);
        __builtin_amdgcn_sched_barrier(0);
    }
    f32x16_t acc, acch;
#pragma unroll
    for (int i = 0; i < 16; ++i) acc[i] = acch[i] = 0.f;
#pragma unroll
    for (int u = 0; u < KTW; ++u) {
        acc = __builtin_amdgcn_mfma_f32_32x32x16_bf16(*(bf16x8_t*)&a[u], *(bf16x8_t*)&b[u], acc, 0, 0, 0);
        acch = __builtin_amdgcn_mfma_f32_32x32x16_bf16(*(bf16x8_t*)&h[u], *(bf16x8_t*)&b[u], acch, 0, 0, 0);
    }
#pragma unroll
    for (int r = 0; r < 16; ++r) red[wave][r][lane] = acc[r];
#pragma unroll
    for (int r = 0; r < 8; ++r) red[wave][16 + r][lane] = o ? acch[8 + r] : acch[r];
    __syncthreads();
    for (int q6 = wave; q6 < 6; q6 += WAVES) {
        float v[4];
#pragma unroll
        for (int j = 0; j < 4; ++j) {
            float s = red[0][4 * q6 + j][lane];
#pragma unroll
            for (int w = 1; w < WAVES; ++w) s += red[w][4 * q6 + j][lane];
            v[j] = s;
        }
        const int nt = q6 < 4 ? tf : th, q = q6 < 4 ? q6 : 2 * o + (q6 - 4);
        skinny_store<EPI_SILU>(v, lane & 31, nt * 32 + 8 * q + 4 * (lane >> 5), 0, nullptr, out, Npad, Npad);
    }
}


template <int WAVES, int EPI, int PRO>
__global__ __launch_bounds__(WAVES * 64, 4) void gemv_small_kernel(
    const u32x4_t* __restrict__ Wp, int KT, int kt_per_split, int kt_per_wave, float* __restrict__ partial,
    uint16_t* __restrict__ out, int Npad, int n_valid, SmallPro pr) {
    __shared__ float red[WAVES][16][64];
    __shared__ float sh[WAVES / 4][4];
    extern __shared__ __attribute__((aligned(16))) u32x4_t xs[];
    const int nt = blockIdx.x, ks = blockIdx.y;
    const int wave = threadIdx.x >> 6, lane = threadIdx.x & 63;
    const int kb0 = ks * kt_per_split;
    int kt0 = kb0 + wave * kt_per_wave;
    int kt1 = min(min(kt0 + kt_per_wave, (ks + 1) * kt_per_split), KT);
    const int n = max(kt1 - kt0, 0);
    constexpr int U = 8;
    const u32x4_t* wp = Wp + ((size_t)nt * KT + kt0) * 64 + lane;
    u32x4_t a[U];
#pragma unroll
    for (int u = 0; u < U; ++u)
        if (u < n) a[u] = __builtin_nontemporal_load(wp + (size_t)u * 64);
    const int kt_base = (PRO == PRO_NORM) ? 0 : kb0;
    if (PRO == PRO_NORM) {
        const int H = KT * 16;
        constexpr int G = WAVES / 4;
        const int g = threadIdx.x >> 8, t = threadIdx.x & 255;
        const size_t kstride = (size_t)MTTS_PFCAP * pr.slab_npad;
        const bool writer = nt == 0 && ks == 0 && pr.x_out != nullptr;
        for (int r0 = 0; r0 < pr.rows; r0 += G) {
            const int r = r0 + g;
            const bool act = r < pr.rows;
            float ss = 0.f;
            const u32x4_t nw0 = (t * 8 < H) ? *(const u32x4_t*)(pr.norm_w + t * 8) : u32x4_t{0u, 0u, 0u, 0u};
#pragma unroll 1
            for (int i0 = t * 8; i0 < H; i0 += 2048) {
                if (!act) break;
                const u32x4_t xo = *(const u32x4_t*)(pr.x_in + (size_t)r * H + i0);
                float v[8];
                if (pr.ksplit > 0) {
                    const float* p0 = pr.slabs + (size_t)r * pr.slab_npad + i0;
                    float4 sa = make_float4(0.f, 0.f, 0.f, 0.f), sb = sa;
                    for (int k0 = 0; k0 < pr.ksplit; k0 += 4) {
                        float4 ta[4], tb[4];
#pragma unroll
                        for (int j = 0; j < 4; ++j) {
                            const float* pk = p0 + (size_t)min(k0 + j, pr.ksplit - 1) * kstride;
                            ta[j] = *(const float4*)pk;
                            tb[j] = *(const float4*)(pk + 4);
                        }
                        if (k0 == 0) { sa = ta[0]; sb = tb[0]; }
#pragma unroll
                        for (int j = 0; j < 4; ++j)
                            if (k0 + j < pr.ksplit && k0 + j > 0) {
                                sa.x += ta[j].x; sa.y += ta[j].y; sa.z += ta[j].z; sa.w += ta[j].w;
                                sb.x += tb[j].x; sb.y += tb[j].y; sb.z += tb[j].z; sb.w += tb[j].w;
                            }
                    }
                    v[0] = rbf(bflo(xo.x) + rbf(sa.x)); v[1] = rbf(bfhi(xo.x) + rbf(sa.y));
                    v[2] = rbf(bflo(xo.y) + rbf(sa.z)); v[3] = rbf(bfhi(xo.y) + rbf(sa.w));
                    v[4] = rbf(bflo(xo.z) + rbf(sb.x)); v[5] = rbf(bfhi(xo.z) + rbf(sb.y));
                    v[6] = rbf(bflo(xo.w) + rbf(sb.z)); v[7] = rbf(bfhi(xo.w) + rbf(sb.w));
                } else {
                    v[0] = bflo(xo.x); v[1] = bfhi(xo.x); v[2] = bflo(xo.y); v[3] = bfhi(xo.y);
                    v[4] = bflo(xo.z); v[5] = bfhi(xo.z); v[6] = bflo(xo.w); v[7] = bfhi(xo.w);
                }
                u32x4_t xn;
                xn.x = pack2(v[0], v[1]); xn.y = pack2(v[2], v[3]); xn.z = pack2(v[4], v[5]); xn.w = pack2(v[6], v[7]);
                if (writer) *(u32x4_t*)(pr.x_out + (size_t)r * H + i0) = xn;
                xs[(size_t)(i0 >> 3) * SMALL_RP + r] = xn;
#pragma unroll
                for (int j = 0; j < 8; ++j) ss += v[j] * v[j];
            }
            ss = wave_sum(ss);
            if ((t & 63) == 0) sh[g][t >> 6] = ss;
            __syncthreads();
            const float tot = sh[g][0] + sh[g][1] + sh[g][2] + sh[g][3];
            __syncthreads();
            const float inv = 1.0f / sqrtf(tot / (float)H + pr.eps);
#pragma unroll 1
            for (int i0 = t * 8; i0 < H; i0 += 2048) {
                if (!act) break;
// ... 211 lines not shown
    int r = idx / n_valid, n = idx % n_valid;
    float s = 0.f;
    for (int k = 0; k < ksplit; ++k) s += partial[((size_t)k * MTTS_PFCAP + r) * Npad + n];
    out[idx] = f2bf(s);
}

static GemmPlan plan_gemm(int Npad, int K, int want_ksplit) {
    GemmPlan p;
    int KT = K / 16, ntiles = Npad / 32;
    int ks = want_ksplit;
    if (ks <= 0) {
        ks = 1;
        while (ntiles * ks < 256 && ks < 8 && KT / (ks * 2) >= 16) ks *= 2;
    }
    p.ksplit = ks;
    p.kt_per_split = (KT + ks - 1) / ks;
    int w = 8;
    while (w > 1 && p.kt_per_split / w < 4) w >>= 1;
    p.waves = w;
    p.kt_per_wave = (p.kt_per_split + w - 1) / w;
    p.depth = 1;
    return p;
}

template <int EPI, int MB>
static void launch_gemm_epi(const GemmPlan& p, const void* Wp, const void* Xp, int K, int Npad, int n_valid,
                            float* partial, uint16_t* out, hipStream_t st) {
    dim3 grid(Npad / 32, p.ksplit);
    int KT = K / 16;
#define MTTS_GEMM_CASE(WV)                                                                            \
    case WV:                                                                                          \
        hipLaunchKernelGGL((gemm_skinny_kernel<WV, EPI, MB>), grid, dim3(WV * 64), 0, st,             \
                           (const u32x4_t*)Wp, (const u32x4_t*)Xp, KT, p.kt_per_split, p.kt_per_wave, \
                           partial, out, Npad, n_valid);                                              \
        break;
    switch (p.waves) {
        MTTS_GEMM_CASE(8)
        MTTS_GEMM_CASE(4)
        MTTS_GEMM_CASE(2)
        MTTS_GEMM_CASE(1)
    }
#undef MTTS_GEMM_CASE
}

template <int EPI>
static void launch_gemm_mb(int mb, const GemmPlan& p, const void* Wp, const void* Xp, int K, int Npad, int n_valid,
                           float* partial, uint16_t* out, hipStream_t st) {
    if (mb <= 1) launch_gemm_epi<EPI, 1>(p, Wp, Xp, K, Npad, n_valid, partial, out, st);
    else if (mb == 2) launch_gemm_epi<EPI, 2>(p, Wp, Xp, K, Npad, n_valid, partial, out, st);
    else launch_gemm_epi<EPI, 4>(p, Wp, Xp, K, Npad, n_valid, partial, out, st);
}

static long long g_depth_launches = 0;
long long mtts_gemm_depth_launches() { return g_depth_launches; }
static bool launch_gemm_depth(int epi, int mb, const GemmPlan& p, const void* Wp, const void* Xp, int K, int Npad,
                              int n_valid, float* partial, uint16_t* out, hipStream_t st) {
    const int KT = K / 16;
    if (!p.depth || mb > 1 || p.waves != 8 || K % 16 || KT != p.ksplit * 8 * p.kt_per_wave || p.kt_per_split != 8 * p.kt_per_wave)
        return false;
    if (epi == EPI_PARTIAL) {
        dim3 grid(Npad / 32, p.ksplit);
#define MTTS_DEPTH_CASE(KTW)                                                                                        \
    case KTW:                                                                                                       \
        hipLaunchKernelGGL((gemm_depth_kernel<8, KTW, EPI_PARTIAL>), grid, dim3(512), 0, st, (const u32x4_t*)Wp,    \
                           (const u32x4_t*)Xp, KT, partial, out, Npad, n_valid);                                    \
        ++g_depth_launches;                                                                                         \
        return true;
        switch (p.kt_per_wave) {
            MTTS_DEPTH_CASE(4)
            MTTS_DEPTH_CASE(12)
        }
#undef MTTS_DEPTH_CASE
        return false;
    }
    if (epi == EPI_SILU && p.ksplit == 1 && p.kt_per_wave == 16 && Npad % 96 == 0 && n_valid == Npad) {
        hipLaunchKernelGGL((gemm_gateup48_kernel<8, 16>), dim3(Npad / 48), dim3(512), 0, st, (const u32x4_t*)Wp,
                           (const u32x4_t*)Xp, KT, out, Npad);
        ++g_depth_launches;
        return true;
    }
    return false;
}

void launch_gemm(int epi, int mb, const GemmPlan& p, const void* Wp, const void* Xp, int K, int Npad, int n_valid,
                 float* partial, uint16_t* out, hipStream_t st) {
    if (launch_gemm_depth(epi, mb, p, Wp, Xp, K, Npad, n_valid, partial, out, st)) return;
    if (epi == EPI_PARTIAL) launch_gemm_mb<EPI_PARTIAL>(mb, p, Wp, Xp, K, Npad, n_valid, partial, out, st);
    else if (epi == EPI_BF16) launch_gemm_mb<EPI_BF16>(mb, p, Wp, Xp, K, Npad, n_valid, partial, out, st);
    else launch_gemm_mb<EPI_SILU>(mb, p, Wp, Xp, K, Npad, n_valid, partial, out, st);
}


int mtts_small_lds_bytes(const GemmPlan& p, int K, int pro) {
    const int kts = pro == PRO_NORM ? K / 16 : p.kt_per_split;
    return kts * 2 * SMALL_RP * 16;
}
template <int EPI, int PRO>
static void launch_small_epi(const GemmPlan& p0, const void* Wp, int K, int Npad, int n_valid, float* partial, uint16_t* out,
                             const SmallPro& pr, hipStream_t st) {
    GemmPlan p = p0;
    if (p.waves < 4) { p.waves = 4; p.kt_per_wave = (p.kt_per_split + 3) / 4; }
    dim3 grid(Npad / 32, p.ksplit);
    const int KT = K / 16;
    const size_t lds = (size_t)mtts_small_lds_bytes(p, K, PRO);
    if (p.waves == 8)
        hipLaunchKernelGGL((gemv_small_kernel<8, EPI, PRO>), grid, dim3(512), lds, st, (const u32x4_t*)Wp, KT, p.kt_per_split,
                           p.kt_per_wave, partial, out, Npad, n_valid, pr);
    else
        hipLaunchKernelGGL((gemv_small_kernel<4, EPI, PRO>), grid, dim3(256), lds, st, (const u32x4_t*)Wp, KT, p.kt_per_split,
                           p.kt_per_wave, partial, out, Npad, n_valid, pr);
}
void launch_gemv_small(int epi, int pro, const GemmPlan& p, const void* Wp, int K, int Npad, int n_valid, float* partial,
                       uint16_t* out, const SmallPro& pr, hipStream_t st) {
    if (epi == EPI_PARTIAL && pro == PRO_NORM) launch_small_epi<EPI_PARTIAL, PRO_NORM>(p, Wp, K, Npad, n_valid, partial, out, pr, st);
    else if (epi == EPI_PARTIAL && pro == PRO_COMBINE) launch_small_epi<EPI_PARTIAL, PRO_COMBINE>(p, Wp, K, Npad, n_valid, partial, out, pr, st);
    else if (epi == EPI_PARTIAL && pro == PRO_ROWS) launch_small_epi<EPI_PARTIAL, PRO_ROWS>(p, Wp, K, Npad, n_valid, partial, out, pr, st);
    else if (epi == EPI_SILU_RM && pro == PRO_NORM) launch_small_epi<EPI_SILU_RM, PRO_NORM>(p, Wp, K, Npad, n_valid, partial, out, pr, st);
    else if (epi == EPI_BF16 && pro == PRO_NORM) launch_small_epi<EPI_BF16, PRO_NORM>(p, Wp, K, Npad, n_valid, partial, out, pr, st);
}

int mtts_tile_ksplit(int Npad, int K, int R) {
    int blocks = ((Npad + 127) / 128) * ((R + 127) / 128), ks = 1;
    while (blocks * ks < 512 && ks < 8 && (K / 16) / (ks * 2) >= 16) ks *= 2;
    return ks;
}
void launch_gemm_tile(int epi, int R, int ksplit, const void* Wp, const void* Xp, int K, int Npad, int n_valid,
                      float* partial, uint16_t* out, hipStream_t st) {
    const int KT = K / 16, ntiles = Npad / 32, rtiles = (R + 31) / 32;
    const int kps = (KT + ksplit - 1) / ksplit;
    dim3 grid((ntiles + 3) / 4, (rtiles + 3) / 4, ksplit);
#define MTTS_TILE_CASE(E)                                                                                     \
    hipLaunchKernelGGL((gemm_tile_kernel<E>), grid, dim3(256), 0, st, (const u32x4_t*)Wp, (const u32x4_t*)Xp, \
                       KT, kps, ntiles, rtiles, partial, out, Npad, n_valid)
    if (epi == EPI_PARTIAL) MTTS_TILE_CASE(EPI_PARTIAL);
    else if (epi == EPI_BF16) MTTS_TILE_CASE(EPI_BF16);
    else MTTS_TILE_CASE(EPI_SILU);
#undef MTTS_TILE_CASE
}

GemmPlan mtts_plan_gemm(int Npad, int K, int want_ksplit) { return plan_gemm(Npad, K, want_ksplit); }
GemmPlan mtts_plan_gemm_forced(int Npad, int K, int ksplit, int waves) {
    GemmPlan p;
    int KT = K / 16;
    p.ksplit = ksplit;
    p.kt_per_split = (KT + ksplit - 1) / ksplit;
    p.waves = waves;
    p.kt_per_wave = (p.kt_per_split + waves - 1) / waves;
    p.depth = 1;
    return p;
}

void launch_pack_weight(const void* src, void* dst, int rows, int cols, int rows_pad, int row_mul, int row_off, hipStream_t st) {
    size_t total = (size_t)rows_pad * cols / 8;
    int blocks = (int)((total + 255) / 256);
    if (blocks > 4096) blocks = 4096;
    hipLaunchKernelGGL(pack_weight_kernel, dim3(blocks), dim3(256), 0, st, (const uint16_t*)src, (uint16_t*)dst, rows,
                       cols, rows_pad, row_mul, row_off);
}
void launch_pack_rows(const void* src, void* dst, int R, int K, int tiles, hipStream_t st) {
    int total = (K / 16) * 64 * tiles;
    hipLaunchKernelGGL(pack_rows_kernel, dim3((total + 255) / 256), dim3(256), 0, st, (const uint16_t*)src,
                       (uint16_t*)dst, R, K, tiles);
}
void launch_reduce_partial_bf16(const float* partial, void* out, int ksplit, int Npad, int n_valid, int R, hipStream_t st) {
    int total = R * n_valid;
    hipLaunchKernelGGL(reduce_partial_bf16_kernel, dim3((total + 255) / 256), dim3(256), 0, st, partial,
                       (uint16_t*)out, ksplit, Npad, n_valid, R);
}
// ... 1 lines not shown
```

### moss-ttsd_amd/csrc/hooks.hip

```cpp
#include "engine.h"

int32_t mtts_k_gemm_bf16(const void* w, const void* x, void* y, int32_t M, int32_t N, int32_t K, int32_t ksplit, void* stream) {
    if (!w || !x || !y || M < 1 || M > MTTS_PFCAP || K % 16 || N < 1) return fail(MTTS_EINVAL, "gemm: need 1<=M<=MTTS_PFCAP, K%%16==0");
    hipStream_t st = S(stream);
    int Npad = round_up(N, 32);
    void *wp = nullptr, *xp = nullptr;
    float* part = nullptr;
    GemmPlan p = mtts_plan_gemm(Npad, K, ksplit);
    p.depth = gemm_depth_env();
    DevBufs hb;
    TRY(hb.get((uint16_t**)&wp, (size_t)Npad * K));
    const bool tiled = M > MTTS_RCAP;
    const int ks = tiled ? (ksplit > 0 ? ksplit : mtts_tile_ksplit(Npad, K, M)) : p.ksplit;
    TRY(hb.get((uint16_t**)&xp, (size_t)MTTS_PFCAP * K));
    TRY(hb.get(&part, (size_t)ks * MTTS_PFCAP * Npad));
    launch_pack_weight(w, wp, N, K, Npad, 1, 0, st);
    const int tiles = (M + 31) / 32;
    launch_pack_rows(x, xp, M, K, tiles == 3 ? 4 : tiles, st);
    if (tiled) launch_gemm_tile(EPI_PARTIAL, M, ks, wp, xp, K, Npad, Npad, part, nullptr, st);
    else launch_gemm(EPI_PARTIAL, tiles, p, wp, xp, K, Npad, Npad, part, nullptr, st);
    launch_reduce_partial_bf16(part, y, ks, Npad, N, M, st);
    HIPCHK(hipGetLastError());
    HIPCHK(hipStreamSynchronize(st));
    return MTTS_OK;
}

int64_t mtts_debug_gemm_depth_launches(void) { return (int64_t)mtts_gemm_depth_launches(); }
int32_t mtts_k_gemm_swiglu_bf16(const void* w, const void* x, void* y, int32_t M, int32_t N, int32_t K, void* stream) {
    if (!w || !x || !y || M < 1 || M > MTTS_RCAP || K % 16 || N < 32 || N % 32) return fail(MTTS_EINVAL, "gemm_swiglu: need 1<=M<=128, K%%16==0, N%%32==0");
    hipStream_t st = S(stream);
    void *wp = nullptr, *xp = nullptr, *op = nullptr;
    GemmPlan p = mtts_plan_gemm(N, K, 1);
    p.depth = gemm_depth_env();
    DevBufs hb;
    const int tiles = (M + 31) / 32, tp = tiles == 3 ? 4 : tiles;
    TRY(hb.get((uint16_t**)&wp, (size_t)N * K));
    TRY(hb.get((uint16_t**)&xp, (size_t)tp * 32 * K));
    TRY(hb.get((uint16_t**)&op, (size_t)tp * 32 * (N / 2)));
    launch_pack_weight(w, wp, N, K, N, 1, 0, st);
    launch_pack_rows(x, xp, M, K, tp, st);
    launch_gemm(EPI_SILU, tiles, p, wp, xp, K, N, N, nullptr, (uint16_t*)op, st);
    launch_unpack_rows(op, y, M, N / 2, st);
    HIPCHK(hipGetLastError());
    HIPCHK(hipStreamSynchronize(st));
    return MTTS_OK;
}

int32_t mtts_k_head_ce(const void* w, const void* x, const int32_t* host_labels, int32_t M, int32_t N, int32_t K, int32_t n_valid,
                       int32_t segments, float* dev_logp, void* stream) {
    if (!w || !x || !host_labels || !dev_logp || M < 1 || M > MTTS_PFCAP || K < 16 || K % 16 || n_valid < 1 || segments < 1 ||
        (segments == 1 ? n_valid > N : N != segments * n_valid))
        return fail(MTTS_EINVAL, "head_ce: need 1<=M<=MTTS_PFCAP, K%%16==0, n_valid<=N (one head) or N==segments*n_valid");
    for (int i = 0; i < M * segments; ++i)
        if (host_labels[i] >= n_valid) return fail(MTTS_EINVAL, "head_ce: label %d outside [0, %d)", host_labels[i], n_valid);
    hipStream_t st = S(stream);
    const int seg_pad = round_up(segments == 1 ? N : n_valid, 32), Mpad = round_up(M, 32);
    uint16_t *wp = nullptr, *xp = nullptr;
    int32_t* lab = nullptr;
    float* part = nullptr;
    DevBufs hb;
    TRY(hb.get(&wp, (size_t)segments * seg_pad * K));
    TRY(hb.get(&xp, (size_t)Mpad * K));
    TRY(hb.get(&lab, (size_t)Mpad * segments, false));
    TRY(hb.get(&part, head_ce_part_elems(M, n_valid, segments), false));
    std::vector<int32_t> hl((size_t)Mpad * segments, -100);
    std::copy(host_labels, host_labels + (size_t)M * segments, hl.begin());
    HIPCHK(hipMemcpyAsync(lab, hl.data(), hl.size() * 4, hipMemcpyHostToDevice, st));
    if (segments == 1) launch_pack_weight(w, wp, N, K, seg_pad, 1, 0, st);
    else
        for (int s = 0; s < segments; ++s)
            launch_pack_weight((const uint16_t*)w + (size_t)s * n_valid * K, wp, n_valid, K, segments * seg_pad, 1, s * seg_pad, st);
    launch_pack_rows(x, xp, M, K, Mpad / 32, st);
    launch_head_ce(wp, xp, M, K, n_valid, segments, lab, segments, 0, part, dev_logp, segments, 0, st);
    HIPCHK(hipGetLastError());
    HIPCHK(hipStreamSynchronize(st));
    return MTTS_OK;
}

int32_t mtts_k_rmsnorm(const void* x, const void* w, void* y, int32_t rows, int32_t n, float eps, void* stream) {
    if (!x || !w || !y || rows < 1 || n < 1) return fail(MTTS_EINVAL, "rmsnorm: bad argument");
    launch_rmsnorm_rows(x, w, y, rows, n, eps, S(stream));
    HIPCHK(hipGetLastError());
    return MTTS_OK;
}

static int k_sample(const void* logits, int32_t rows, int32_t vocab, const void* bitmap, const MttsSamplerCfg* cfg,
                    int32_t mask_id, uint64_t seed, int32_t step, int32_t channel, int32_t* dev_tokens, float* dev_logp, void* stream) {
    if (!logits || !cfg || !dev_tokens || rows < 1 || vocab < 1 || channel < 0 || channel > 7) return fail(MTTS_EINVAL, "sample: bad argument");
    hipStream_t st = S(stream);
    MttsSamplerCfg h[8];
    for (int i = 0; i < 8; ++i) h[i] = *cfg;
    MttsSamplerCfg* d = nullptr;
    int32_t *err = nullptr, *dec = nullptr;
    if (rows > MTTS_RCAP) return fail(MTTS_EINVAL, "sample: at most 128 rows");
    DevBufs hb;
    TRY(hb.get(&d, 8));
    TRY(hb.get(&err, 1));
    TRY(hb.get(&dec, (size_t)rows * 8));
    HIPCHK(hipMemcpy(d, h, sizeof(h), hipMemcpyHostToDevice));
    SampleScratch sc;
    TRY(alloc_scratch(hb, sc, rows, vocab));
    if (dev_logp) TRY(alloc_lp_scratch(hb, sc, rows));
    launch_sample_single(logits, rows, vocab, (const uint32_t*)bitmap, (vocab + 31) / 32, d, mask_id, seed, step, channel, dec, err, sc,
                         full_cap_for(vocab), dev_logp ? 1 : 0, st);
    HIPCHK(hipGetLastError());
    HIPCHK(hipStreamSynchronize(st));
    std::vector<int32_t> hd((size_t)rows * 8);
    int32_t herr = 0;
    HIPCHK(hipMemcpy(hd.data(), dec, hd.size() * 4, hipMemcpyDeviceToHost));
    HIPCHK(hipMemcpy(&herr, err, 4, hipMemcpyDeviceToHost));
    std::vector<int32_t> outv(rows);
    for (int r = 0; r < rows; ++r) outv[r] = hd[(size_t)r * 8 + channel];
    HIPCHK(hipMemcpy(dev_tokens, outv.data(), rows * 4, hipMemcpyHostToDevice));
    if (dev_logp) {
        std::vector<float> hl((size_t)rows * 8), outl(rows);
        HIPCHK(hipMemcpy(hl.data(), sc.lp, hl.size() * 4, hipMemcpyDeviceToHost));
        for (int r = 0; r < rows; ++r) outl[r] = hl[(size_t)r * 8 + channel];
        HIPCHK(hipMemcpy(dev_logp, outl.data(), rows * 4, hipMemcpyHostToDevice));
    }
    if (herr) return fail(MTTS_EINVAL, "sample: more than 4096 candidate tokens");
    return MTTS_OK;
}

int32_t mtts_k_sample(const void* logits, int32_t rows, int32_t vocab, const void* bitmap, const MttsSamplerCfg* cfg,
// ... 218 lines not shown
    if (kv_len < 1 || kv_len > limit) return fail(MTTS_EINVAL, "kv_len %d outside 1..%d", kv_len, limit);
    e->max_steps = std::min(e->max_steps, e->steps_issued + cap - kv_len);
    std::vector<SeqState> ss(MTTS_RCAP);
    HIPCHK(hipMemcpy(ss.data(), e->d_seqs, ss.size() * sizeof(SeqState), hipMemcpyDeviceToHost));
    for (int b = 0; b < e->B; ++b) { ss[b].kv_len = kv_len; e->n_real[b] = kv_len - e->steps_issued; }
    e->max_real = kv_len - e->steps_issued;
    HIPCHK(hipMemcpy(e->d_seqs, ss.data(), ss.size() * sizeof(SeqState), hipMemcpyHostToDevice));
    launch_fill_random_bf16(e->kcache, e->layer_stride * e->L, 0x1234u, nullptr);
    launch_fill_random_bf16(e->vcache, e->layer_stride * e->L, 0x9876u, nullptr);
    if (e->kpack) launch_kv_seal_all(e->kcache, e->vcache, e->kpack, e->vpack, e->total_pages, e->nkv, e->L, nullptr, nullptr);
    HIPCHK(hipDeviceSynchronize());
    return MTTS_OK;
}

int32_t mtts_k_attn_bench(MttsEngine* e, int32_t phase, int32_t iters, float* avg_ms, int64_t* bytes_per_launch) {
    if (!e || !e->began || phase < ATTN_ALL || phase > ATTN_ROW || iters < 1 || !avg_ms) return fail(MTTS_EINVAL, "attn_bench: bad argument");
    if (e->f32) return fail(MTTS_EINVAL, "measurement hook of the bf16 engine");
    HIPCHK(hipSetDevice(e->device));
    HIPCHK(hipDeviceSynchronize());
    const float scale = 1.0f / sqrtf((float)MTTS_HD);
    const int R = round_up(e->B, 32);
    const int len_bound = e->max_real + e->steps_issued + 1;
    const int pages_bound = (len_bound + MTTS_PAGE - 1) / MTTS_PAGE;
    if (phase == ATTN_ROW) {
        if (attn_row_prepare()) return fail(MTTS_EINVAL, "attn_row_kernel: the dynamic LDS limit could not be raised");
        const QkvFuse f0{e->partial, e->p_qkv.ksplit, e->qkv_rows, nullptr, nullptr, nullptr, nullptr, 0.f};
        for (int n = 0; n < e->L; ++n) {
            const KvPack pk = layer_pack(e, n, pages_bound);
            if (!attn_row_fits(e->nq / e->nkv, &f0, (pk.k || pk.v) ? &pk : nullptr, pages_bound))
                return fail(MTTS_EINVAL, "attn_bench: the whole-row kernel does not take this shape");
        }
    }
    hipEvent_t e0, e1;
    hipEventCreate(&e0); hipEventCreate(&e1);
    auto run = [&](int n) {
        for (int i = 0; i < n; ++i) {
            const int layer = i % e->L;
            uint16_t* kc = (uint16_t*)e->kcache + e->layer_stride * layer;
            uint16_t* vc = (uint16_t*)e->vcache + e->layer_stride * layer;
            const QkvFuse fz{e->partial, e->p_qkv.ksplit, e->qkv_rows, (const uint16_t*)e->layers[layer].qn,
                             (const uint16_t*)e->layers[layer].kn, e->rope_cos, e->rope_sin, e->cfg.rms_norm_eps};
            const KvPack pk = layer_pack(e, layer, pages_bound);
            launch_attn(e->qbuf, kc, vc, e->d_page_table, e->d_meta, e->scores, e->stats, e->opart, e->attn_p, R, pages_bound,
                        e->max_pages, e->total_pages, e->nchunks_max, e->nq, e->nkv, scale, (phase == ATTN_ROW || e->B * pages_bound <= e->fuse_qkv_max) ? &fz : nullptr, (AttnPhase)phase, nullptr,
                        (pk.k || pk.v) ? &pk : nullptr);
        }
    };
    run(e->L);
    hipEventRecord(e0, nullptr);
    run(iters);
    hipEventRecord(e1, nullptr);
    HIPCHK(hipEventSynchronize(e1));
    float ms = 0;
    hipEventElapsedTime(&ms, e0, e1);
    *avg_ms = ms / iters;
    if (bytes_per_launch) {
        std::vector<RowMeta> m(MTTS_RCAP);
        HIPCHK(hipMemcpy(m.data(), e->d_meta, m.size() * sizeof(RowMeta), hipMemcpyDeviceToHost));
        int64_t tok = 0;
        for (int b = 0; b < R; ++b) if (m[b].seq >= 0) tok += m[b].pos + 1;
        *bytes_per_launch = phase == ATTN_COMBINE ? 0 : tok * e->nkv * MTTS_HD * 2 * ((phase == ATTN_ALL || phase == ATTN_ROW) ? 2 : 1);
    }
    hipEventDestroy(e0); hipEventDestroy(e1);
    return MTTS_OK;
}

int32_t mtts_k_gemm_bench(int32_t N, int32_t K, int32_t epi, int32_t ksplit, int32_t waves, int32_t copies,
                                     int32_t iters, float* avg_us) {
    if (N % 32 || K % 16 || copies < 1 || iters < 1 || !avg_us) return fail(MTTS_EINVAL, "gemm_bench: bad argument");
    const int tile_rows = waves < 0 ? -waves : 0;
    if (tile_rows > MTTS_PFCAP) return fail(MTTS_EINVAL, "gemm_bench: at most MTTS_PFCAP rows");
    GemmPlan p = (ksplit > 0 && waves > 0) ? mtts_plan_gemm_forced(N, K, ksplit, waves) : mtts_plan_gemm(N, K, tile_rows ? std::max(ksplit, 1) : ksplit);
    if (tile_rows) p.ksplit = std::max(ksplit, 1);
    p.depth = gemm_depth_env();
    DevBufs hb;
    std::vector<uint16_t*> w(copies, nullptr);
    for (auto& q : w) { TRY(hb.get(&q, (size_t)N * K, false)); HIPCHK(hipMemset(q, 0x3c, (size_t)N * K * 2)); }
    uint16_t *x = nullptr, *out = nullptr;
    float* part = nullptr;
    TRY(hb.get(&x, (size_t)MTTS_PFCAP * K, false));
    HIPCHK(hipMemset(x, 0x3c, (size_t)MTTS_PFCAP * K * 2));
    TRY(hb.get(&out, (size_t)MTTS_PFCAP * N));
    TRY(hb.get(&part, (size_t)p.ksplit * MTTS_PFCAP * N));
    hipEvent_t e0, e1;
    hipEventCreate(&e0); hipEventCreate(&e1);
    auto go = [&](int i) {
        if (tile_rows) launch_gemm_tile(epi, tile_rows, p.ksplit, w[i % copies], x, K, N, N, part, out, nullptr);
        else launch_gemm(epi, 1, p, w[i % copies], x, K, N, N, part, out, nullptr);
    };
    for (int i = 0; i < copies; ++i) go(i);
    HIPCHK(hipDeviceSynchronize());
    hipEventRecord(e0, nullptr);
    for (int i = 0; i < iters; ++i) go(i);
    hipEventRecord(e1, nullptr);
    HIPCHK(hipEventSynchronize(e1));
    float ms = 0;
    hipEventElapsedTime(&ms, e0, e1);
    *avg_us = ms * 1000.f / iters;
    hipEventDestroy(e0); hipEventDestroy(e1);
    return MTTS_OK;
}
```

### moss-ttsd_amd/csrc/launch.h

```cpp
#pragma once
#include <type_traits>

#include "../../include/mtts.h"
#include "common.h"

enum { EPI_PARTIAL = 0, EPI_BF16 = 1, EPI_SILU = 2,
       EPI_SILU_RM = 3 };
struct GemmPlan {
    int waves, ksplit, kt_per_split, kt_per_wave;
    int depth;
};
GemmPlan mtts_plan_gemm(int Npad, int K, int want_ksplit);
GemmPlan mtts_plan_gemm_forced(int Npad, int K, int ksplit, int waves);
void launch_gemm(int epi, int mb, const GemmPlan& p, const void* Wp, const void* Xp, int K, int Npad, int n_valid,
                 float* partial, uint16_t* out, hipStream_t st);
int mtts_tile_ksplit(int Npad, int K, int R);
void launch_gemm_tile(int epi, int R, int ksplit, const void* Wp, const void* Xp, int K, int Npad, int n_valid,
                      float* partial, uint16_t* out, hipStream_t st);
int mtts_small_lds_bytes(const GemmPlan& p, int K, int pro);
void launch_gemv_small(int epi, int pro, const GemmPlan& p, const void* Wp, int K, int Npad, int n_valid, float* partial,
                       uint16_t* out, const SmallPro& pr, hipStream_t st);
long long mtts_gemm_depth_launches();
void launch_pack_weight(const void* src, void* dst, int rows, int cols, int rows_pad, int row_mul, int row_off, hipStream_t st);
void launch_pack_rows(const void* src, void* dst, int R, int K, int tiles, hipStream_t st);
void launch_reduce_partial_bf16(const float* partial, void* out, int ksplit, int Npad, int n_valid, int R, hipStream_t st);

struct PageEdits { int32_t n; int32_t idx[31]; int32_t val[31]; };
static_assert(sizeof(PageEdits) == 252, "PageEdits is a kernel argument: one 32-bit count + 31 (index, value) pairs");
void launch_embed_norm(const int32_t* tokens, const RowMeta* meta, const uint16_t* const* tables, const void* norm_w,
                       void* x, void* xn_packed, int R, int H, float eps, hipStream_t st);
void launch_resid_norm(const float* partial, int ksplit, int Npad, void* x, const void* norm_w, void* xn_packed,
                       void* hlast, const RowMeta* meta, int R, int H, float eps, hipStream_t st);
void launch_qkv_post(const float* partial, int ksplit, int Npad, const RowMeta* meta, const void* qnw, const void* knw,
                     const void* cosb, const void* sinb, void* qbuf, void* kcache, void* vcache,
                     const int32_t* page_table, int max_pages, int total_pages, int R, int nq, int nkv, float eps,
                     hipStream_t st);
void launch_rmsnorm_rows(const void* x, const void* w, void* y, int rows, int n, float eps, hipStream_t st);
void launch_fill_random_bf16(void* p, size_t n, uint32_t seed, hipStream_t st);
void launch_set_pages(int32_t* table, const PageEdits& ed, hipStream_t st);
void launch_fork(void* kc, void* vc, size_t layer_bytes, size_t head_bytes, int blk_bytes, int L, int nkv, const ForkJob& job,
                 hipStream_t st);
void launch_pack_kv_pages(const void* K, const void* V, void* kcache, void* vcache, const int32_t* page_table, const int32_t* lens,
                          int S, int Lmax, int nkv, int max_pages, int total_pages, hipStream_t st);
void launch_bf16_to_f32(const void* a, float* b, size_t n, hipStream_t st);
void launch_unpack_rows(const void* packed, void* out, int R, int K, hipStream_t st);

enum AttnPhase { ATTN_ALL = 0, ATTN_SCORES = 1, ATTN_PV = 2, ATTN_COMBINE = 3,
                 ATTN_ROW = 4,
                 ATTN_PF_SCORES = 11, ATTN_PF_PV = 12, ATTN_PF_COMBINE = 13 };
int launch_attn(const void* qbuf, void* kcache, void* vcache, const int32_t* page_table,
                const RowMeta* meta, void* scores, float* stats, float* opart, void* out_packed, int R,
                int pages_bound, int max_pages, int total_pages, int nchunks_max, int nq, int nkv, float scale,
                const QkvFuse* fuse, AttnPhase phase, hipStream_t st, const KvPack* pack = nullptr);
bool attn_row_fits(int G, const QkvFuse* fuse, const KvPack* pack, int pages_bound);
int attn_row_prepare();
int attn_row_lds_limit();
long long mtts_attn_row_launches();
void launch_kv_seal_rows(const void* kcache, const void* vcache, void* kpack, void* vpack, const int32_t* page_table,
                         const RowMeta* meta, int R, int max_pages, int total_pages, int nkv, int L, unsigned long long* cnt, hipStream_t st);
void launch_kv_seal_all(const void* kcache, const void* vcache, void* kpack, void* vpack, int total_pages, int nkv, int L,
                        unsigned long long* cnt, hipStream_t st);
void launch_kv_seal_pages(const void* raw, void* pk, int npages, int as_k, hipStream_t st);
void launch_kv_pack_count(const void* kpack, const void* vpack, const int32_t* page_table, const int32_t* complete, int B, int max_pages,
                          int total_pages, int nkv, int L, unsigned long long* out, hipStream_t st);

struct SeqState {
    int32_t nas;
    int32_t unfinished;
    int32_t kv_len;
    int32_t step;
    int32_t base_length;
    int32_t max_length;
    int32_t row_id;
    int32_t active;
    uint64_t seed;
};

struct LoopState {
    int32_t step;
    int32_t done;
    int32_t continuous;
    int32_t B;
    int32_t error;
    int32_t gen_cap;
    int32_t forced_draw;
    int32_t logits_f32;
};
static_assert(sizeof(SeqState) == 40 && std::is_trivially_copyable<SeqState>::value, "SeqState layout");
static_assert(sizeof(LoopState) == 32 && std::is_trivially_copyable<LoopState>::value, "LoopState layout");

#define SAMP_CAND 4096
#define SAMP_NS 32
struct SampleScratch {
    uint32_t* hist = nullptr;
    float* slice_val = nullptr;
    int32_t* slice_idx = nullptr;
    float* cand_val = nullptr;
    int32_t* cand_idx = nullptr;
// ... 49 lines not shown
```

### moss-ttsd_amd/mtts/capi.py

```python
from __future__ import annotations

import ctypes as C
import os

_HERE = os.path.dirname(os.path.abspath(__file__))
LIB_PATH = os.path.join(os.path.dirname(_HERE), "lib", "libmtts.so")


class MttsConfig(C.Structure):
    _fields_ = [(n, C.c_int32) for n in (
        "vocab_size", "hidden_size", "intermediate_size", "num_hidden_layers", "num_attention_heads",
        "num_key_value_heads", "head_dim", "channels", "speech_vocab_size", "speech_pad_token",
        "speech_range_lo", "speech_range_hi", "eos_token_id", "max_position")] + [
        ("rms_norm_eps", C.c_float), ("max_batch", C.c_int32), ("max_seq_len", C.c_int32), ("kv_pool_pages", C.c_int32), ("dtype", C.c_int32)]


class MttsSamplerCfg(C.Structure):
    _fields_ = [("do_sample", C.c_int32), ("top_k", C.c_int32), ("top_p", C.c_float),
                ("one_minus_top_p", C.c_float), ("temperature", C.c_float), ("repetition_penalty", C.c_float)]


class MttsCodecConfig(C.Structure):
    _fields_ = [(n, C.c_int32) for n in (
        "nq", "codebook_size", "rvq_dim", "quant_out_dim",
        "adapter_layers", "adapter_dim", "adapter_heads", "adapter_ffn", "adapter_max_pos", "up_stride",
        "dec_layers", "dec_dim", "dec_heads", "dec_ffn", "dec_max_pos", "mel_bins",
        "voc_dim", "voc_inter", "voc_layers", "n_fft", "hop",
        "mel_n_fft", "mel_hop", "mel_frames", "enc_layers", "enc_dim", "enc_heads", "enc_ffn", "enc_max_pos",
        "sem_adapter_layers", "pre_rvq_layers", "down_pool")]


class MttsError(RuntimeError):
    def __init__(self, msg, code=0):
        super().__init__(msg)
        self.code = code


EINVAL = -1
ENOMEM = -3
ESTATE = -4


_lib = None

_SIGS = {
    "mtts_last_error": (C.c_char_p, []),
    "mtts_version": (C.c_int32, []),
    "mtts_engine_create": (C.c_int32, [C.POINTER(MttsConfig), C.c_int32, C.POINTER(C.c_void_p)]),
    "mtts_engine_destroy": (C.c_int32, [C.c_void_p]),
    "mtts_bind_weight": (C.c_int32, [C.c_void_p, C.c_char_p, C.c_void_p, C.c_int64, C.c_int64, C.c_void_p]),
    "mtts_bind_rope": (C.c_int32, [C.c_void_p, C.c_void_p, C.c_void_p, C.c_int32, C.c_void_p]),
    "mtts_weights_ready": (C.c_int32, [C.c_void_p]),
    "mtts_generate": (C.c_int32, [C.c_void_p, C.c_void_p, C.c_void_p, C.c_int32, C.c_int32, C.c_int32,
                                  C.POINTER(MttsSamplerCfg), C.c_uint64, C.c_void_p, C.c_int32,
                                  C.POINTER(C.c_int32), C.c_void_p, C.c_int32, C.c_void_p, C.c_void_p]),
    "mtts_begin": (C.c_int32, [C.c_void_p, C.c_void_p, C.c_void_p, C.c_int32, C.c_int32, C.c_int32,
                               C.POINTER(MttsSamplerCfg), C.c_uint64, C.c_void_p]),
    "mtts_step": (C.c_int32, [C.c_void_p, C.c_int32, C.c_void_p]),
    "mtts_sync_state": (C.c_int32, [C.c_void_p, C.POINTER(C.c_int32), C.POINTER(C.c_int32), C.c_void_p]),
    "mtts_read_generated": (C.c_int32, [C.c_void_p, C.c_void_p, C.c_int32, C.POINTER(C.c_int32)]),
    "mtts_set_output_scores": (C.c_int32, [C.c_void_p, C.c_int32]),
    "mtts_read_scores": (C.c_int32, [C.c_void_p, C.c_void_p, C.c_int32, C.POINTER(C.c_int32)]),
    "mtts_slot_read_scores": (C.c_int32, [C.c_void_p, C.c_int32, C.c_void_p, C.c_int32, C.POINTER(C.c_int32)]),
    "mtts_score": (C.c_int32, [C.c_void_p, C.c_void_p, C.c_void_p, C.c_void_p, C.c_int32, C.c_int32, C.c_void_p, C.c_void_p]),
    "mtts_read_logits": (C.c_int32, [C.c_void_p, C.c_void_p, C.c_void_p, C.c_void_p]),
    "mtts_read_logits_f32": (C.c_int32, [C.c_void_p, C.c_void_p, C.c_void_p, C.c_void_p]),
    "mtts_sched_open": (C.c_int32, [C.c_void_p, C.c_int32, C.c_int32, C.POINTER(MttsSamplerCfg), C.c_void_p]),
    "mtts_slot_submit": (C.c_int32, [C.c_void_p, C.c_int32, C.c_void_p, C.c_int32, C.c_int32, C.c_uint64, C.c_void_p]),
    "mtts_slot_submit_row": (C.c_int32, [C.c_void_p, C.c_int32, C.c_void_p, C.c_int32, C.c_int32, C.c_uint64, C.c_int32, C.c_void_p]),
    "mtts_set_row_ids": (C.c_int32, [C.c_void_p, C.c_void_p, C.c_int32]),
    "mtts_set_takes": (C.c_int32, [C.c_void_p, C.c_int32]),
    "mtts_slot_fork": (C.c_int32, [C.c_void_p, C.c_int32, C.c_int32, C.c_uint64, C.c_int32, C.c_void_p]),
    "mtts_slot_states": (C.c_int32, [C.c_void_p, C.c_void_p, C.c_void_p]),
    "mtts_slot_read": (C.c_int32, [C.c_void_p, C.c_int32, C.c_void_p, C.c_int32, C.POINTER(C.c_int32)]),
    "mtts_read_seq_state": (C.c_int32, [C.c_void_p, C.c_void_p, C.c_void_p, C.c_void_p, C.c_void_p]),
    "mtts_slot_evict": (C.c_int32, [C.c_void_p, C.c_int32, C.c_void_p]),
    "mtts_kv_pool_state": (C.c_int32, [C.c_void_p, C.POINTER(C.c_int32), C.POINTER(C.c_int32), C.POINTER(C.c_int32)]),
    "mtts_read_page_table": (C.c_int32, [C.c_void_p, C.c_void_p, C.c_void_p]),
    "mtts_set_forced_mode": (C.c_int32, [C.c_void_p, C.c_int32]),
    "mtts_debug_read_device_page_table": (C.c_int32, [C.c_void_p, C.c_void_p, C.c_void_p]),
    "mtts_export_codes": (C.c_int32, [C.c_void_p, C.c_int32, C.c_int32, C.c_void_p, C.c_void_p]),
    "mtts_profile_enable": (C.c_int32, [C.c_void_p, C.c_int32]),
    "mtts_profile_read": (C.c_int32, [C.c_void_p, C.c_int32, C.POINTER(C.c_double), C.POINTER(C.c_int64),
                                      C.POINTER(C.c_int64)]),
    "mtts_debug_set_kv_len": (C.c_int32, [C.c_void_p, C.c_int32]),
    "mtts_debug_kv_pack_stats": (C.c_int32, [C.c_void_p, C.c_void_p]),
    "mtts_k_kv_seal": (C.c_int32, [C.c_void_p, C.c_int32, C.c_void_p, C.c_int32, C.c_void_p]),
    "mtts_k_attn_bench": (C.c_int32, [C.c_void_p, C.c_int32, C.c_int32, C.POINTER(C.c_float), C.POINTER(C.c_int64)]),
    "mtts_k_gemm_bench": (C.c_int32, [C.c_int32] * 7 + [C.POINTER(C.c_float)]),
    "mtts_k_gemm_bf16": (C.c_int32, [C.c_void_p, C.c_void_p, C.c_void_p, C.c_int32, C.c_int32, C.c_int32,
                                     C.c_int32, C.c_void_p]),
    "mtts_debug_gemm_depth_launches": (C.c_int64, []),
    "mtts_debug_attn_row_launches": (C.c_int64, []),
    "mtts_k_attn_section": (C.c_int32, [C.c_void_p, C.c_int32] + [C.c_void_p] * 4 + [C.c_float] + [C.c_void_p] * 4 +
                            [C.c_int32] * 6 + [C.c_void_p] * 6),
    "mtts_k_gemm_swiglu_bf16": (C.c_int32, [C.c_void_p, C.c_void_p, C.c_void_p, C.c_int32, C.c_int32, C.c_int32, C.c_void_p]),
    "mtts_k_rmsnorm": (C.c_int32, [C.c_void_p, C.c_void_p, C.c_void_p, C.c_int32, C.c_int32, C.c_float, C.c_void_p]),
    "mtts_k_rope_kvwrite": (C.c_int32, [C.c_void_p] * 6 + [C.c_int32, C.c_int32, C.c_int32, C.c_float] + [C.c_void_p] * 4),
    "mtts_k_paged_attn_decode": (C.c_int32, [C.c_void_p] * 5 + [C.c_int32] * 4 + [C.c_void_p, C.c_void_p]),
    "mtts_k_head_ce": (C.c_int32, [C.c_void_p, C.c_void_p, C.c_void_p] + [C.c_int32] * 5 + [C.c_void_p, C.c_void_p]),
    "mtts_k_sample": (C.c_int32, [C.c_void_p, C.c_int32, C.c_int32, C.c_void_p, C.POINTER(MttsSamplerCfg),
                                  C.c_int32, C.c_uint64, C.c_int32, C.c_int32, C.c_void_p, C.c_void_p]),
    "mtts_k_sample_scores": (C.c_int32, [C.c_void_p, C.c_int32, C.c_int32, C.c_void_p, C.POINTER(MttsSamplerCfg),
                                         C.c_int32, C.c_uint64, C.c_int32, C.c_int32, C.c_void_p, C.c_void_p, C.c_void_p]),
    "mtts_codec_last_error": (C.c_char_p, []),
    "mtts_codec_create": (C.c_int32, [C.POINTER(MttsCodecConfig), C.c_int32, C.POINTER(C.c_void_p)]),
    "mtts_codec_destroy": (C.c_int32, [C.c_void_p]),
    "mtts_codec_bind": (C.c_int32, [C.c_void_p, C.c_char_p, C.c_void_p, C.c_int64, C.c_void_p]),
    "mtts_codec_detokenize": (C.c_int32, [C.c_void_p, C.c_void_p, C.c_void_p, C.c_int32, C.c_int32, C.c_void_p, C.c_void_p]),
    "mtts_codec_detokenize_async": (C.c_int32, [C.c_void_p, C.c_void_p, C.c_void_p, C.c_int32, C.c_int32, C.c_void_p, C.c_void_p]),
    "mtts_codec_check": (C.c_int32, [C.c_void_p, C.c_void_p]),
    "mtts_codec_tokenize": (C.c_int32, [C.c_void_p, C.c_void_p, C.c_void_p, C.c_int32, C.c_int32, C.c_void_p, C.c_void_p, C.c_void_p]),
    "mtts_k_gemm_f32": (C.c_int32, [C.c_void_p, C.c_void_p, C.c_void_p, C.c_void_p, C.c_int32, C.c_int32, C.c_int32,
                                    C.c_int32, C.c_void_p]),
    "mtts_k_gemm_planes_bench": (C.c_int32, [C.c_int32, C.c_int32, C.c_int32, C.c_int32, C.c_int32, C.c_int32,
                                             C.POINTER(C.c_float), C.POINTER(C.c_int32)]),
}


def exported_symbols():
    return sorted(_SIGS)


def lib():
    global _lib
    if _lib is None:
        if not os.path.exists(LIB_PATH):
            raise MttsError(f"{LIB_PATH} is missing: build it with `python moss-ttsd_amd/build.py` "
                            "(hipcc --offload-arch=gfx950); there is no CPU fallback")
        L = C.CDLL(LIB_PATH)
        for name, (res, args) in _SIGS.items():
            fn = getattr(L, name)
            fn.restype = res
            fn.argtypes = args
        _lib = L
    return _lib


def check(rc):
    if rc != 0:
        raise MttsError(f"libmtts error {rc}: {lib().mtts_last_error().decode()}", rc)
```

### moss-ttsd_amd/mtts/engine.py

```python
from __future__ import annotations

import ctypes as C

import numpy as np
import torch

from . import capi


def sampler_cfgs(layers=None, do_samples=None):
    arr = (capi.MttsSamplerCfg * 8)()
    for i in range(8):
        lc = (layers[i] if layers and i < len(layers) else {}) or {}
        s = arr[i]
        s.do_sample = 1 if (do_samples and do_samples[i]) else 0
        s.top_k = int(lc.get("top_k") or 0)
        tp = lc.get("top_p")
        s.top_p = float(tp) if tp is not None else 0.0
        s.one_minus_top_p = float(np.float32(1.0 - tp)) if tp is not None else 0.0
        t = lc.get("temperature")
        s.temperature = float(t) if t is not None else 0.0
        rp = lc.get("repetition_penalty")
        s.repetition_penalty = float(rp) if rp is not None else 0.0
    return arr
# ... 162 lines not shown
        return buf[:n.value]

    def read_logits(self):
        V0, Vs = self.cfg["vocab_size"], self.cfg["speech_vocab_size"]
        if self.dtype != "bf16":
            l0 = np.zeros((self._B, V0), dtype=np.float32)
            l17 = np.zeros((7, self._B, Vs), dtype=np.float32)
            capi.check(self.lib.mtts_read_logits_f32(self._h, l0.ctypes.data, l17.ctypes.data, None))
            return l0, l17
        l0 = np.zeros((self._B, V0), dtype=np.uint16)
        l17 = np.zeros((7, self._B, Vs), dtype=np.uint16)
        capi.check(self.lib.mtts_read_logits(self._h, l0.ctypes.data, l17.ctypes.data, None))
        f = lambda u: (u.astype(np.uint32) << 16).view(np.float32)
        return f(l0), f(l17)

    def sched_open(self, slots, gen_cap, layers=None, do_samples=None, output_scores=False):
        self._B = int(slots)
        self.set_output_scores(output_scores)
        capi.check(self.lib.mtts_sched_open(self._h, int(slots), int(gen_cap), sampler_cfgs(layers, do_samples), None))

    def submit(self, slot, ids, max_length, seed=0, row_id=0):
        ids = np.ascontiguousarray(ids, dtype=np.int64)
        assert ids.ndim == 2 and ids.shape[1] == 8
        capi.check(self.lib.mtts_slot_submit_row(self._h, int(slot), ids.ctypes.data, ids.shape[0], int(max_length),
                                                 C.c_uint64(seed), int(row_id), None))

    def fork(self, src, dst, seed=0, row_id=0):
        capi.check(self.lib.mtts_slot_fork(self._h, int(src), int(dst), C.c_uint64(seed), int(row_id), None))

    def slot_states(self):
        st = np.zeros((self._B, 4), dtype=np.int32)
        capi.check(self.lib.mtts_slot_states(self._h, st.ctypes.data, None))
        return st

    def slot_read(self, slot, capacity):
        buf = np.zeros((int(capacity), 8), dtype=np.int64)
        n = C.c_int32(0)
        capi.check(self.lib.mtts_slot_read(self._h, int(slot), buf.ctypes.data, int(capacity), C.byref(n)))
        return buf[:n.value].copy()

    def slot_read_scores(self, slot, capacity):
        buf = np.zeros((max(int(capacity), 1), 8), dtype=np.float32)
        n = C.c_int32(0)
        capi.check(self.lib.mtts_slot_read_scores(self._h, int(slot), buf.ctypes.data, buf.shape[0], C.byref(n)))
        return buf[:n.value].copy()

    def evict(self, slot):
        capi.check(self.lib.mtts_slot_evict(self._h, int(slot), None))

    def kv_pool_state(self):
        a, b, c = C.c_int32(0), C.c_int32(0), C.c_int32(0)
        capi.check(self.lib.mtts_kv_pool_state(self._h, C.byref(a), C.byref(b), C.byref(c)))
        return a.value, b.value, c.value

    def page_table(self, max_batch):
        _, _, mp = self.kv_pool_state()
        t = np.zeros((int(max_batch), mp), dtype=np.int32)
        n = np.zeros(int(max_batch), dtype=np.int32)
        capi.check(self.lib.mtts_read_page_table(self._h, t.ctypes.data, n.ctypes.data))
        return t, n

    def device_page_table(self, max_batch):
        _, _, mp = self.kv_pool_state()
        t = np.zeros((int(max_batch), mp), dtype=np.int32)
        capi.check(self.lib.mtts_debug_read_device_page_table(self._h, t.ctypes.data, None))
        return t

    def seq_state(self):
        a, u, k = (np.zeros(self._B, dtype=np.int32) for _ in range(3))
        capi.check(self.lib.mtts_read_seq_state(self._h, a.ctypes.data, u.ctypes.data, k.ctypes.data, None))
        return a, u, k

    def export_codes(self, first, n, stream=None):
        out = torch.empty(8, self._B, n, dtype=torch.int64, device=self.device)
        sp = C.c_void_p(stream.cuda_stream) if stream is not None else None
        capi.check(self.lib.mtts_export_codes(self._h, int(first), int(n), out.data_ptr(), sp))
        return out

    def kv_pack_stats(self):
        o = np.zeros(6, dtype=np.int64)
        capi.check(self.lib.mtts_debug_kv_pack_stats(self._h, o.ctypes.data))
        return dict(zip(("k_pages", "k_unsealed", "v_pages", "v_unsealed", "k_layers_on", "v_layers_on"), (int(x) for x in o)))

    def debug_set_kv_len(self, n):
        capi.check(self.lib.mtts_debug_set_kv_len(self._h, int(n)))

    def attn_bench(self, phase, iters=112):
        ms, by = C.c_float(0), C.c_int64(0)
        capi.check(self.lib.mtts_k_attn_bench(self._h, int(phase), int(iters), C.byref(ms), C.byref(by)))
        return ms.value, by.value

    def profile(self, on=True):
        capi.check(self.lib.mtts_profile_enable(self._h, 1 if on else 0))

    def profile_read(self, which):
        ms, n, by = C.c_double(0), C.c_int64(0), C.c_int64(0)
        capi.check(self.lib.mtts_profile_read(self._h, which, C.byref(ms), C.byref(n), C.byref(by)))
        return ms.value, n.value, by.value
```

Baseline: 81820 codec_tokens/s.

## Store down-proj and head weights in sealed exponent-dictionary compressed form

```diff
diff --git a/include/mtts.h b/include/mtts.h
--- a/include/mtts.h
+++ b/include/mtts.h
@@ -105,6 +105,7 @@
 
 int32_t mtts_debug_set_kv_len(MttsEngine* e, int32_t kv_len);
 int32_t mtts_debug_kv_pack_stats(MttsEngine* e, int64_t* out6);
+int32_t mtts_debug_w_seal_stats(MttsEngine* e, int64_t* out10);
 int32_t mtts_k_attn_bench(MttsEngine* e, int32_t phase, int32_t iters, float* avg_ms, int64_t* bytes_per_launch);
 int32_t mtts_k_gemm_bench(int32_t N, int32_t K, int32_t epi, int32_t ksplit, int32_t waves, int32_t copies,
                           int32_t iters, float* avg_us);
@@ -112,6 +113,11 @@
 int32_t mtts_k_gemm_bf16(const void* dev_w, const void* dev_x, void* dev_y,
                          int32_t M, int32_t N, int32_t K, int32_t ksplit, void* stream);
 int64_t mtts_debug_gemm_depth_launches(void);
+int64_t mtts_debug_w_seal_launches(void);
+int32_t mtts_k_gemm_head_bf16(const void* dev_w, const void* dev_x, void* dev_y, int32_t M, int32_t N, int32_t n_valid,
+                              int32_t K, void* stream);
+int32_t mtts_k_w_seal(const void* dev_w, int32_t N, int32_t K, int32_t T, void* dev_packed, void* dev_sealed,
+                      int64_t* counts2, void* stream);
 int64_t mtts_debug_attn_row_launches(void);
 int32_t mtts_k_attn_section(const float* dev_slabs, int32_t ksplit, const void* dev_qnw, const void* dev_knw, const void* dev_cos,
                             const void* dev_sin, float eps, const void* dev_k, const void* dev_v, const int32_t* host_lens,
diff --git a/moss-ttsd_amd/csrc/attn.hip b/moss-ttsd_amd/csrc/attn.hip
--- a/moss-ttsd_amd/csrc/attn.hip
+++ b/moss-ttsd_amd/csrc/attn.hip
@@ -1,4 +1,5 @@
 #include "launch.h"
+#include "seal.h"
 #include <algorithm>
 #include <atomic>
 #include <cstdlib>
@@ -11,82 +12,6 @@
 #define PK_OCC(PK)
 #endif
 
-__device__ __forceinline__ uint32_t u4c(const u32x4_t& v, int c) { return c == 0 ? v.x : c == 1 ? v.y : c == 2 ? v.z : v.w; }
-__device__ __forceinline__ void pk_unit(const u32x4_t* pk, int j, uint32_t w[4]) {
-    const uint32_t L0 = u4c(pk[j >> 1], 2 * (j & 1)), L1 = u4c(pk[j >> 1], 2 * (j & 1) + 1);
-    const uint32_t N = u4c(pk[8 + (j >> 2)], j & 3);
-    const uint32_t lo = pk[12].x, hi = pk[12].y;
-    const uint32_t HA = ((N & 0x08080808u) << 4) | __builtin_amdgcn_perm(hi, lo, N & 0x07070707u);
-    const uint32_t HB = (N & 0x80808080u) | __builtin_amdgcn_perm(hi, lo, (N >> 4) & 0x07070707u);
-    w[0] = __builtin_amdgcn_perm(HA, L0, 0x05010400u);
-    w[1] = __builtin_amdgcn_perm(HA, L0, 0x07030602u);
-    w[2] = __builtin_amdgcn_perm(HB, L1, 0x05010400u);
-    w[3] = __builtin_amdgcn_perm(HB, L1, 0x07030602u);
-}
-
-__host__ __device__ constexpr int pk_order(int i) { return i == 0 ? 12 : (i - 1) % 3 == 0 ? 8 + (i - 1) / 3 : 2 * ((i - 1) / 3) + (i - 1) % 3 - 1; }
-__device__ bool seal_encode(const u32x4_t (&v)[16], u32x4_t* __restrict__ pk, uint32_t spare, bool unfit) {
-    unsigned long long b0 = 0ull, b1 = 0ull;
-#pragma unroll
-    for (int j = 0; j < 16; ++j)
-#pragma unroll
-        for (int c = 0; c < 4; ++c)
-#pragma unroll
-            for (int h = 0; h < 2; ++h) {
-                const uint32_t e = (u4c(v[j], c) >> (8 + 16 * h)) & 0x7fu;
-                if (e & 64u) b1 |= 1ull << (e & 63u);
-                else b0 |= 1ull << e;
-            }
-    const int n0 = __popcll(b0), n = n0 + __popcll(b1);
-    if (n > 8 || unfit) {
-        pk[12 * 64] = u32x4_t{0u, 0u, spare, 1u};
-        return false;
-    }
-    unsigned long long dict = 0ull;
-    {
-        unsigned long long t0 = b0, t1 = b1;
-        for (int i = 0; i < n; ++i) {
-            uint32_t e;
-            if (t0) { e = __ffsll((long long)t0) - 1; t0 &= t0 - 1; }
-            else { e = 64 + __ffsll((long long)t1) - 1; t1 &= t1 - 1; }
-            dict |= (unsigned long long)e << (8 * i);
-        }
-    }
-    auto code = [&](uint32_t half) -> uint32_t {
-        const uint32_t e = (half >> 8) & 0x7fu;
-        const uint32_t rank = (e & 64u) ? n0 + __popcll(b1 & ((1ull << (e & 63u)) - 1ull)) : __popcll(b0 & ((1ull << e) - 1ull));
-        return ((half >> 12) & 8u) | rank;
-    };
-    uint32_t lowp[32], nib[16];
-#pragma unroll
-    for (int j = 0; j < 16; ++j) {
-        uint32_t N = 0u;
-#pragma unroll
-        for (int g = 0; g < 2; ++g) {
-            uint32_t L = 0u;
-#pragma unroll
-            for (int k = 0; k < 4; ++k) {
-                const uint32_t half = (u4c(v[j], 2 * g + (k >> 1)) >> (16 * (k & 1))) & 0xffffu;
-                L |= (half & 0xffu) << (8 * k);
-                N |= code(half) << (8 * k + 4 * g);
-            }
-            lowp[2 * j + g] = L;
-        }
-        nib[j] = N;
-    }
-#pragma unroll
-    for (int u = 0; u < 8; ++u) pk[u * 64] = u32x4_t{lowp[4 * u], lowp[4 * u + 1], lowp[4 * u + 2], lowp[4 * u + 3]};
-#pragma unroll
-    for (int u = 0; u < 4; ++u) pk[(8 + u) * 64] = u32x4_t{nib[4 * u], nib[4 * u + 1], nib[4 * u + 2], nib[4 * u + 3]};
-    pk[12 * 64] = u32x4_t{(uint32_t)dict, (uint32_t)(dict >> 32), spare, 0u};
-    return true;
-}
-__device__ bool seal_lane(const u32x4_t* __restrict__ raw, u32x4_t* __restrict__ pk) {
-    u32x4_t v[16];
-#pragma unroll
-    for (int j = 0; j < 16; ++j) v[j] = raw[j * 64];
-    return seal_encode(v, pk, 0u, false);
-}
 __device__ bool seal_lane_k(const u32x4_t* __restrict__ raw, u32x4_t* __restrict__ pk, uint8_t* __restrict__ lds, int lane) {
     u32x4_t v[16];
 #pragma unroll
diff --git a/moss-ttsd_amd/csrc/engine.h b/moss-ttsd_amd/csrc/engine.h
--- a/moss-ttsd_amd/csrc/engine.h
+++ b/moss-ttsd_amd/csrc/engine.h
@@ -33,6 +33,14 @@
     return (g && atoi(g) == 0) ? 0 : 1;
 }
 
+static inline int w_seal_env() {
+    const char* g = getenv("MTTS_W_SEAL");
+    return g ? std::min(std::max(atoi(g), 0), 2) : 1;
+}
+static inline bool w_seal_pays(int mode, unsigned long long sealed, unsigned long long unsealed) {
+    return mode == 2 || unsealed * 8 <= sealed + unsealed;
+}
+
 template <typename T>
 static int dalloc(T** p, size_t n, bool zero = true) {
     HIPCHK(hipMalloc((void**)p, n * sizeof(T)));
@@ -113,6 +121,7 @@
 
 struct Layer {
     void *wqkv = nullptr, *wo = nullptr, *wgu = nullptr, *wd = nullptr;
+    void* wd_s = nullptr;
     void *ln_in = nullptr, *ln_post = nullptr, *qn = nullptr, *kn = nullptr;
     int bound = 0;
 };
@@ -141,6 +150,12 @@
     void *x2 = nullptr, *act_rm = nullptr;
     int small_rows = SMALL_RP;
     int gemm_depth = 1;
+    int w_seal = 1;
+    bool w_seal_done = false;
+    void *head0_s = nullptr, *heads17_s = nullptr;
+    unsigned long long w_seal_cnt[3][2] = {{0, 0}, {0, 0}, {0, 0}};
+    char w_seal_on[3] = {0, 0, 0};
+    size_t w_seal_bytes = 0;
     void *x = nullptr, *xn = nullptr, *attn_p = nullptr, *act_p = nullptr, *qbuf = nullptr, *hlast = nullptr, *xh = nullptr;
     void *logits0 = nullptr, *logits17 = nullptr, *join_logits0 = nullptr, *join_logits17 = nullptr;
     void* scores = nullptr;
@@ -202,7 +217,7 @@
     int max_real = 0;
     uint64_t seed = 0;
     bool began = false, has_forced = false;
-    struct StepGraph { int B, pages, forced, ch0, scores, row; hipGraphExec_t exec; };
+    struct StepGraph { int B, pages, forced, ch0, scores, row, wseal; hipGraphExec_t exec; };
     std::vector<StepGraph> graphs;
     hipStream_t cap_stream = nullptr;
     bool use_graphs = true;
@@ -230,6 +245,10 @@
     return e->attn_row == 2 || attn_row_auto(e->B, e->nkv, pages_bound, e->n_cus);
 }
 
+static inline int w_seal_mask(const MttsEngine* e) {
+    return e->w_seal_on[0] | e->w_seal_on[1] << 1 | e->w_seal_on[2] << 2;
+}
+
 static inline KvPack layer_pack(MttsEngine* e, int n, int pages_bound) {
     KvPack pk{nullptr, nullptr};
     if (e->B * pages_bound < e->pack_min_work) return pk;
diff --git a/moss-ttsd_amd/csrc/engine.hip b/moss-ttsd_amd/csrc/engine.hip
--- a/moss-ttsd_amd/csrc/engine.hip
+++ b/moss-ttsd_amd/csrc/engine.hip
@@ -141,6 +141,8 @@
     return MTTS_OK;
 }
 
+static void drop_sealed_weights(MttsEngine* e);
+static int weights_bound(MttsEngine* e);
 static void drop_graphs(MttsEngine* e) {
     for (auto& g : e->graphs) hipGraphExecDestroy(g.exec);
     e->graphs.clear();
@@ -187,6 +189,7 @@
     }
     if (const char* g = getenv("MTTS_SMALL_ROWS")) e->small_rows = std::min(std::max(atoi(g), 0), SMALL_RP);
     e->gemm_depth = gemm_depth_env();
+    e->w_seal = e->gemm_depth ? w_seal_env() : 0;
     e->H = c->hidden_size; e->I = c->intermediate_size; e->L = c->num_hidden_layers;
     e->nq = c->num_attention_heads; e->nkv = c->num_key_value_heads;
     e->V0 = c->vocab_size; e->Vs = c->speech_vocab_size;
@@ -379,6 +382,7 @@
     WeightSlot w;
     TRY(resolve_weight(e, name_c, w));
     if (!w.bound) return MTTS_OK;
+    if (w.pack_to) drop_sealed_weights(e);
     const bool shape_ok = w.cols == 1 ? (rows == w.rows && cols == 1) || (rows == 1 && cols == w.rows) : rows == w.rows && cols == w.cols;
     if (!shape_ok)
         return fail(MTTS_EINVAL, "%s: expected [%lld,%lld] got [%lld,%lld]", name_c, (long long)w.rows, (long long)w.cols, (long long)rows, (long long)cols);
@@ -413,7 +417,74 @@
     return bind_rope_tables(e, e->rope_cos, e->rope_sin, cosb, sinb, rows, S(stream));
 }
 
+static void drop_sealed_weights(MttsEngine* e) {
+    if (!e->w_seal_done && !e->head0_s && !e->heads17_s) return;
+    hipDeviceSynchronize();
+    for (auto& l : e->layers) e->mem.release(l.wd_s);
+    e->mem.release(e->head0_s);
+    e->mem.release(e->heads17_s);
+    memset(e->w_seal_cnt, 0, sizeof(e->w_seal_cnt));
+    memset(e->w_seal_on, 0, sizeof(e->w_seal_on));
+    e->w_seal_bytes = 0;
+    e->w_seal_done = false;
+}
+
+static int seal_weights(MttsEngine* e) {
+    if (e->w_seal_done) return MTTS_OK;
+    e->w_seal_done = true;
+    if (e->f32 || !e->w_seal) return MTTS_OK;
+    HIPCHK(hipSetDevice(e->device));
+    HIPCHK(hipDeviceSynchronize());
+    const int H = e->H, I = e->I, Hp = round_up(H, 32);
+    const struct { int epi; const GemmPlan* p; int K, Npad, n_valid, per_layer; } g[3] = {
+        {EPI_PARTIAL, &e->p_d, I, Hp, Hp, 1}, {EPI_BF16, &e->p_h0, H, e->V0_pad, e->V0, 0}, {EPI_BF16, &e->p_h17, H, 7 * e->Vs_pad, 7 * e->Vs_pad, 0}};
+    int T[3];
+    size_t need = 0;
+    for (int i = 0; i < 3; ++i) {
+        T[i] = mtts_w_seal_depth(g[i].epi, *g[i].p, g[i].K, g[i].Npad, g[i].n_valid);
+        if (T[i]) need += mtts_w_seal_bytes(g[i].Npad, g[i].K, T[i]) * (g[i].per_layer ? e->L : 1);
+    }
+    if (!need) return MTTS_OK;
+    size_t free_b = 0, total_b = 0;
+    if (hipMemGetInfo(&free_b, &total_b) != hipSuccess || need + ((size_t)8 << 30) > free_b) {
+        fprintf(stderr, "mtts: sealed weights off: %.1f GB needed, %.1f GB free (8 GB kept for the run)\n", need / 1e9, free_b / 1e9);
+        return MTTS_OK;
+    }
+    DevBufs tmp;
+    unsigned long long* d_cnt = nullptr;
+    TRY(tmp.get(&d_cnt, 6));
+    for (int i = 0; i < 3; ++i) {
+        if (!T[i]) continue;
+        const size_t bytes = mtts_w_seal_bytes(g[i].Npad, g[i].K, T[i]);
+        if (g[i].per_layer)
+            for (auto& l : e->layers) {
+                TRY(e->mem.get((uint8_t**)&l.wd_s, bytes, false));
+                launch_w_seal(l.wd, l.wd_s, g[i].Npad, g[i].K, T[i], d_cnt + 2 * i, nullptr);
+            }
+        else {
+            void*& dst = i == 1 ? e->head0_s : e->heads17_s;
+            TRY(e->mem.get((uint8_t**)&dst, bytes, false));
+            launch_w_seal(i == 1 ? e->head0 : e->heads17, dst, g[i].Npad, g[i].K, T[i], d_cnt + 2 * i, nullptr);
+        }
+    }
+    HIPCHK(hipGetLastError());
+    HIPCHK(hipMemcpy(e->w_seal_cnt, d_cnt, sizeof(e->w_seal_cnt), hipMemcpyDeviceToHost));
+    for (int i = 0; i < 3; ++i) {
+        if (!T[i]) continue;
+        e->w_seal_on[i] = w_seal_pays(e->w_seal, e->w_seal_cnt[i][0], e->w_seal_cnt[i][1]);
+        if (e->w_seal_on[i]) { e->w_seal_bytes += mtts_w_seal_bytes(g[i].Npad, g[i].K, T[i]) * (g[i].per_layer ? e->L : 1); continue; }
+        if (i == 0) for (auto& l : e->layers) e->mem.release(l.wd_s);
+        else e->mem.release(i == 1 ? e->head0_s : e->heads17_s);
+    }
+    return MTTS_OK;
+}
+
 int32_t mtts_weights_ready(MttsEngine* e) {
+    TRY(weights_bound(e));
+    return seal_weights(e);
+}
+
+static int weights_bound(MttsEngine* e) {
     if (!e) return fail(MTTS_EINVAL, "null engine");
     if (e->emb_bound != 0xff) return fail(MTTS_ESTATE, "embedding tables missing (mask %x)", e->emb_bound);
     if (!e->norm_bound) return fail(MTTS_ESTATE, "final norm missing");
@@ -550,7 +621,7 @@
             launch_gemm_tile(EPI_PARTIAL, R, ks_d, l.wd, e->act_p, I, Hp, Hp, e->partial, nullptr, st);
         } else {
             launch_gemm(EPI_SILU, mb, e->p_gu, l.wgu, e->xn, H, 2 * I, 2 * I, nullptr, (uint16_t*)e->act_p, st);
-            launch_gemm(EPI_PARTIAL, mb, e->p_d, l.wd, e->act_p, I, Hp, Hp, e->partial, nullptr, st);
+            launch_gemm(EPI_PARTIAL, mb, e->p_d, l.wd, e->act_p, I, Hp, Hp, e->partial, nullptr, st, l.wd_s);
         }
         const bool lastl = (n == e->L - 1);
         const void* nw = lastl ? e->final_norm : e->layers[n + 1].ln_in;
@@ -566,8 +637,9 @@
             launch_pack_rows(e->hlast, e->xh, e->B, H, hmb, st);
             xin = e->xh;
         }
-        launch_gemm(EPI_BF16, hmb, e->p_h0, e->head0, xin, H, e->V0_pad, e->V0, nullptr, (uint16_t*)e->logits0, st);
-        launch_gemm(EPI_BF16, hmb, e->p_h17, e->heads17, xin, H, 7 * e->Vs_pad, 7 * e->Vs_pad, nullptr, (uint16_t*)e->logits17, st);
+        launch_gemm(EPI_BF16, hmb, e->p_h0, e->head0, xin, H, e->V0_pad, e->V0, nullptr, (uint16_t*)e->logits0, st, heads == 1 ? e->head0_s : nullptr);
+        launch_gemm(EPI_BF16, hmb, e->p_h17, e->heads17, xin, H, 7 * e->Vs_pad, 7 * e->Vs_pad, nullptr, (uint16_t*)e->logits17, st,
+                    heads == 1 ? e->heads17_s : nullptr);
     }
     HIPCHK(hipGetLastError());
     return MTTS_OK;
@@ -805,9 +877,10 @@
 }
 
 static int step_graph(MttsEngine* e, int pages, hipGraphExec_t* out) {
-    const int forced = e->has_forced ? 1 : 0, row = attn_row_shape(e, pages) ? 1 : 0;
+    const int forced = e->has_forced ? 1 : 0, row = attn_row_shape(e, pages) ? 1 : 0, wseal = w_seal_mask(e);
     for (auto& g : e->graphs)
-        if (g.B == e->B && g.pages == pages && g.forced == forced && g.ch0 == e->ch0_sampled && g.scores == e->scores_on && g.row == row) {
+        if (g.B == e->B && g.pages == pages && g.forced == forced && g.ch0 == e->ch0_sampled && g.scores == e->scores_on && g.row == row &&
+            g.wseal == wseal) {
             *out = g.exec;
             return MTTS_OK;
         }
@@ -823,7 +896,7 @@
     hipError_t ie = hipGraphInstantiate(&exec, g, nullptr, nullptr, 0);
     hipGraphDestroy(g);
     HIPCHK(ie);
-    e->graphs.push_back({e->B, pages, forced, e->ch0_sampled, e->scores_on, row, exec});
+    e->graphs.push_back({e->B, pages, forced, e->ch0_sampled, e->scores_on, row, wseal, exec});
     *out = exec;
     return MTTS_OK;
 }
diff --git a/moss-ttsd_amd/csrc/gemm.hip b/moss-ttsd_amd/csrc/gemm.hip
--- a/moss-ttsd_amd/csrc/gemm.hip
+++ b/moss-ttsd_amd/csrc/gemm.hip
@@ -1,4 +1,5 @@
 #include "launch.h"
+#include "seal.h"
 
 
 template <int WAVES, int EPI, int MB>
@@ -196,6 +197,105 @@
         }
         const int nt = q6 < 4 ? tf : th, q = q6 < 4 ? q6 : 2 * o + (q6 - 4);
         skinny_store<EPI_SILU>(v, lane & 31, nt * 32 + 8 * q + 4 * (lane >> 5), 0, nullptr, out, Npad, Npad);
+    }
+}
+
+template <int T> __host__ __device__ constexpr int ws_units() { return T == 16 ? MTTS_PKU : 10; }
+template <int T> __host__ __device__ constexpr int ws_slot(int id) { return T == 16 ? id : id < 6 ? id : id < 11 ? id - 2 : 9; }
+
+template <int T>
+__global__ __launch_bounds__(64) void w_seal_kernel(const u32x4_t* __restrict__ Wp, u32x4_t* __restrict__ Ws, int KT,
+                                                    unsigned long long* __restrict__ cnt) {
+    __shared__ u32x4_t stage[MTTS_PKU * 64];
+    const int lane = threadIdx.x, KB = KT / T;
+    const u32x4_t* raw = Wp + ((size_t)blockIdx.y * KT + (size_t)blockIdx.x * T) * 64 + lane;
+    u32x4_t* dst = Ws + ((size_t)blockIdx.y * KB + blockIdx.x) * (ws_units<T>() * 64) + lane;
+    bool fit;
+    if (T == 16) fit = seal_lane(raw, dst);
+    else {
+        u32x4_t v[16];
+#pragma unroll
+        for (int j = 0; j < T; ++j) v[j] = raw[j * 64];
+        const uint32_t f = (v[0].x & 0xffffu) * 0x10001u;
+#pragma unroll
+        for (int j = T; j < 16; ++j) v[j] = u32x4_t{f, f, f, f};
+#pragma unroll
+        for (int u = 0; u < MTTS_PKU; ++u) stage[u * 64 + lane] = u32x4_t{0u, 0u, 0u, 0u};
+        fit = seal_encode(v, stage + lane, 0u, false);
+#pragma unroll
+        for (int u = 0; u < MTTS_PKU; ++u)
+            if (u < 6 || (u >= 8 && u != 11)) dst[ws_slot<T>(u) * 64] = stage[u * 64 + lane];
+    }
+    const bool all = !__any(!fit);
+    if (cnt && lane == 0) atomicAdd(cnt + (all ? 0 : 1), 1ull);
+}
+
+template <int T>
+__device__ __forceinline__ void ws_request(const u32x4_t* __restrict__ p, u32x4_t (&pk)[MTTS_PKU]) {
+#pragma unroll
+    for (int i = 0; i < ws_units<T>(); ++i) {
+        pk[pk_order(i)] = __builtin_nontemporal_load(p + ws_slot<T>(pk_order(i)) * 64);
+        __builtin_amdgcn_sched_barrier(0);
+    }
+}
+template <int T>
+__device__ __forceinline__ void ws_keep(const u32x4_t (&pk)[MTTS_PKU]) {
+#pragma unroll
+    for (int i = 1; i < ws_units<T>(); ++i) asm volatile("" ::"v"(pk[pk_order(i)]));
+}
+__device__ __forceinline__ u32x4_t ws_tile(const u32x4_t (&pk)[MTTS_PKU], int u) {
+    uint32_t w[4];
+    pk_unit(pk, u, w);
+    return u32x4_t{w[0], w[1], w[2], w[3]};
+}
+
+template <int WAVES, int KTW, int EPI>
+__global__ __launch_bounds__(WAVES * 64) void gemm_sealed_kernel(
+    const u32x4_t* __restrict__ Ws, const u32x4_t* __restrict__ Wp, const u32x4_t* __restrict__ Xp, int KT,
+    float* __restrict__ partial, uint16_t* __restrict__ out, int Npad, int n_valid) {
+    __shared__ float red[WAVES][16][64];
+    const int nt = blockIdx.x, ks = blockIdx.y;
+    const int wave = threadIdx.x >> 6, lane = threadIdx.x & 63;
+    const int kb = ks * WAVES + wave, KB = KT / KTW;
+    const u32x4_t* sp = Ws + ((size_t)nt * KB + kb) * (ws_units<KTW>() * 64) + lane;
+    const u32x4_t* xp = Xp + (size_t)kb * KTW * 64 + lane;
+    u32x4_t b[KTW], pk[MTTS_PKU];
+#pragma unroll
+    for (int u = 0; u < KTW; ++u) b[u] = xp[(size_t)u * 64];
+    __builtin_amdgcn_sched_barrier(0);
+    ws_request<KTW>(sp, pk);
+    f32x16_t acc;
+#pragma unroll
+    for (int i = 0; i < 16; ++i) acc[i] = 0.f;
+    if (__any(pk[12].w != 0u)) {
+        const u32x4_t* wp = Wp + ((size_t)nt * KT + (size_t)kb * KTW) * 64 + lane;
+        u32x4_t a[KTW];
+#pragma unroll
+        for (int u = 0; u < KTW; ++u) a[u] = __builtin_nontemporal_load(wp + (size_t)u * 64);
+        ws_keep<KTW>(pk);
+#pragma unroll
+        for (int u = 0; u < KTW; ++u)
+            acc = __builtin_amdgcn_mfma_f32_32x32x16_bf16(*(bf16x8_t*)&a[u], *(bf16x8_t*)&b[u], acc, 0, 0, 0);
+    } else {
+#pragma unroll
+        for (int u = 0; u < KTW; ++u) {
+            u32x4_t a = ws_tile(pk, u);
+            acc = __builtin_amdgcn_mfma_f32_32x32x16_bf16(*(bf16x8_t*)&a, *(bf16x8_t*)&b[u], acc, 0, 0, 0);
+        }
+    }
+#pragma unroll
+    for (int r = 0; r < 16; ++r) red[wave][r][lane] = acc[r];
+    __syncthreads();
+    for (int q = wave; q < 4; q += WAVES) {
+        float v[4];
+#pragma unroll
+        for (int j = 0; j < 4; ++j) {
+            float s = red[0][4 * q + j][lane];
+#pragma unroll
+            for (int w = 1; w < WAVES; ++w) s += red[w][4 * q + j][lane];
+            v[j] = s;
+        }
+        skinny_store<EPI>(v, lane & 31, nt * 32 + 8 * q + 4 * (lane >> 5), ks, partial, out, Npad, n_valid);
     }
 }
 
@@ -573,8 +673,42 @@
     return false;
 }
 
+int mtts_w_seal_depth(int epi, const GemmPlan& p, int K, int Npad, int n_valid) {
+    const int KT = K / 16;
+    if (p.waves != 8 || K % 16 || KT != p.ksplit * 8 * p.kt_per_wave || p.kt_per_split != 8 * p.kt_per_wave) return 0;
+    if (epi == EPI_PARTIAL && p.kt_per_wave == 12) return 12;
+    if (epi == EPI_BF16 && p.ksplit == 1 && p.kt_per_wave == 16) return 16;
+    (void)Npad; (void)n_valid;
+    return 0;
+}
+size_t mtts_w_seal_bytes(int Npad, int K, int T) { return (size_t)(Npad / 32) * (K / 16 / T) * (T == 16 ? MTTS_PKU : 10) * 64 * 16; }
+void launch_w_seal(const void* Wp, void* Ws, int Npad, int K, int T, unsigned long long* cnt, hipStream_t st) {
+    const int KT = K / 16;
+    const dim3 grid(KT / T, Npad / 32);
+    if (T == 16) hipLaunchKernelGGL(w_seal_kernel<16>, grid, dim3(64), 0, st, (const u32x4_t*)Wp, (u32x4_t*)Ws, KT, cnt);
+    else hipLaunchKernelGGL(w_seal_kernel<12>, grid, dim3(64), 0, st, (const u32x4_t*)Wp, (u32x4_t*)Ws, KT, cnt);
+}
+static long long g_sealed_launches = 0;
+long long mtts_w_seal_launches() { return g_sealed_launches; }
+static bool launch_gemm_sealed(int epi, int mb, const GemmPlan& p, const void* Ws, const void* Wp, const void* Xp, int K,
+                               int Npad, int n_valid, float* partial, uint16_t* out, hipStream_t st) {
+    if (!Ws || !p.depth || mb > 1) return false;
+    const int T = mtts_w_seal_depth(epi, p, K, Npad, n_valid), KT = K / 16;
+    if (!T) return false;
+    if (epi == EPI_PARTIAL)
+        hipLaunchKernelGGL((gemm_sealed_kernel<8, 12, EPI_PARTIAL>), dim3(Npad / 32, p.ksplit), dim3(512), 0, st, (const u32x4_t*)Ws,
+                           (const u32x4_t*)Wp, (const u32x4_t*)Xp, KT, partial, out, Npad, n_valid);
+    else
+        hipLaunchKernelGGL((gemm_sealed_kernel<8, 16, EPI_BF16>), dim3(Npad / 32, 1), dim3(512), 0, st, (const u32x4_t*)Ws,
+                           (const u32x4_t*)Wp, (const u32x4_t*)Xp, KT, partial, out, Npad, n_valid);
+    ++g_sealed_launches;
+    ++g_depth_launches;
+    return true;
+}
+
 void launch_gemm(int epi, int mb, const GemmPlan& p, const void* Wp, const void* Xp, int K, int Npad, int n_valid,
-                 float* partial, uint16_t* out, hipStream_t st) {
+                 float* partial, uint16_t* out, hipStream_t st, const void* Ws) {
+    if (launch_gemm_sealed(epi, mb, p, Ws, Wp, Xp, K, Npad, n_valid, partial, out, st)) return;
     if (launch_gemm_depth(epi, mb, p, Wp, Xp, K, Npad, n_valid, partial, out, st)) return;
     if (epi == EPI_PARTIAL) launch_gemm_mb<EPI_PARTIAL>(mb, p, Wp, Xp, K, Npad, n_valid, partial, out, st);
     else if (epi == EPI_BF16) launch_gemm_mb<EPI_BF16>(mb, p, Wp, Xp, K, Npad, n_valid, partial, out, st);
diff --git a/moss-ttsd_amd/csrc/hooks.hip b/moss-ttsd_amd/csrc/hooks.hip
--- a/moss-ttsd_amd/csrc/hooks.hip
+++ b/moss-ttsd_amd/csrc/hooks.hip
@@ -1,4 +1,21 @@
 #include "engine.h"
+
+static int hook_w_seal(DevBufs& hb, int epi, int tiles, const GemmPlan& p, const void* wp, int K, int Npad, int n_valid,
+                       hipStream_t st, void** ws) {
+    *ws = nullptr;
+    const int mode = p.depth ? w_seal_env() : 0, T = mtts_w_seal_depth(epi, p, K, Npad, n_valid);
+    if (!mode || tiles != 1 || !T) return MTTS_OK;
+    uint8_t* s = nullptr;
+    unsigned long long *d_cnt = nullptr, h_cnt[2];
+    TRY(hb.get(&s, mtts_w_seal_bytes(Npad, K, T), false));
+    TRY(hb.get(&d_cnt, 2));
+    launch_w_seal(wp, s, Npad, K, T, d_cnt, st);
+    HIPCHK(hipGetLastError());
+    HIPCHK(hipMemcpyAsync(h_cnt, d_cnt, sizeof(h_cnt), hipMemcpyDeviceToHost, st));
+    HIPCHK(hipStreamSynchronize(st));
+    if (w_seal_pays(mode, h_cnt[0], h_cnt[1])) *ws = s;
+    return MTTS_OK;
+}
 
 int32_t mtts_k_gemm_bf16(const void* w, const void* x, void* y, int32_t M, int32_t N, int32_t K, int32_t ksplit, void* stream) {
     if (!w || !x || !y || M < 1 || M > MTTS_PFCAP || K % 16 || N < 1) return fail(MTTS_EINVAL, "gemm: need 1<=M<=MTTS_PFCAP, K%%16==0");
@@ -17,8 +34,10 @@
     launch_pack_weight(w, wp, N, K, Npad, 1, 0, st);
     const int tiles = (M + 31) / 32;
     launch_pack_rows(x, xp, M, K, tiles == 3 ? 4 : tiles, st);
+    void* ws = nullptr;
+    if (!tiled) TRY(hook_w_seal(hb, EPI_PARTIAL, tiles, p, wp, K, Npad, Npad, st, &ws));
     if (tiled) launch_gemm_tile(EPI_PARTIAL, M, ks, wp, xp, K, Npad, Npad, part, nullptr, st);
-    else launch_gemm(EPI_PARTIAL, tiles, p, wp, xp, K, Npad, Npad, part, nullptr, st);
+    else launch_gemm(EPI_PARTIAL, tiles, p, wp, xp, K, Npad, Npad, part, nullptr, st, ws);
     launch_reduce_partial_bf16(part, y, ks, Npad, N, M, st);
     HIPCHK(hipGetLastError());
     HIPCHK(hipStreamSynchronize(st));
@@ -26,6 +45,60 @@
 }
 
 int64_t mtts_debug_gemm_depth_launches(void) { return (int64_t)mtts_gemm_depth_launches(); }
+int64_t mtts_debug_w_seal_launches(void) { return (int64_t)mtts_w_seal_launches(); }
+
+int32_t mtts_k_gemm_head_bf16(const void* w, const void* x, void* y, int32_t M, int32_t N, int32_t n_valid, int32_t K, void* stream) {
+    if (!w || !x || !y || M < 1 || M > MTTS_RCAP || K % 16 || N < 1 || n_valid < 1 || n_valid > N) return fail(MTTS_EINVAL, "gemm_head: need 1<=M<=128, K%%16==0, 1<=n_valid<=N");
+    hipStream_t st = S(stream);
+    const int Npad = round_up(N, 32), tiles = (M + 31) / 32, tp = tiles == 3 ? 4 : tiles;
+    void *wp = nullptr, *xp = nullptr, *ws = nullptr;
+    GemmPlan p = mtts_plan_gemm(Npad, K, 1);
+    p.depth = gemm_depth_env();
+    DevBufs hb;
+    TRY(hb.get((uint16_t**)&wp, (size_t)Npad * K));
+    TRY(hb.get((uint16_t**)&xp, (size_t)tp * 32 * K));
+    launch_pack_weight(w, wp, N, K, Npad, 1, 0, st);
+    launch_pack_rows(x, xp, M, K, tp, st);
+    TRY(hook_w_seal(hb, EPI_BF16, tiles, p, wp, K, Npad, n_valid, st, &ws));
+    uint16_t* yp = nullptr;
+    TRY(hb.get(&yp, (size_t)tp * 32 * Npad));
+    launch_gemm(EPI_BF16, tiles, p, wp, xp, K, Npad, n_valid, nullptr, yp, st, ws);
+    HIPCHK(hipGetLastError());
+    HIPCHK(hipMemcpyAsync(y, yp, (size_t)M * Npad * 2, hipMemcpyDeviceToDevice, st));
+    HIPCHK(hipStreamSynchronize(st));
+    return MTTS_OK;
+}
+
+int32_t mtts_k_w_seal(const void* w, int32_t N, int32_t K, int32_t T, void* dev_packed, void* dev_sealed, int64_t* counts2, void* stream) {
+    if (!w || !dev_sealed || !counts2 || N < 32 || N % 32 || (T != 16 && T != 12) || K < 16 * T || K % (16 * T))
+        return fail(MTTS_EINVAL, "w_seal: need N%%32==0, T 16 or 12, K%%(16 T)==0");
+    hipStream_t st = S(stream);
+    DevBufs hb;
+    uint16_t* wp = nullptr;
+    unsigned long long *d_cnt = nullptr, h_cnt[2];
+    TRY(hb.get(&wp, (size_t)N * K));
+    TRY(hb.get(&d_cnt, 2));
+    launch_pack_weight(w, wp, N, K, N, 1, 0, st);
+    launch_w_seal(wp, dev_sealed, N, K, T, d_cnt, st);
+    HIPCHK(hipGetLastError());
+    if (dev_packed) HIPCHK(hipMemcpyAsync(dev_packed, wp, (size_t)N * K * 2, hipMemcpyDeviceToDevice, st));
+    HIPCHK(hipMemcpyAsync(h_cnt, d_cnt, sizeof(h_cnt), hipMemcpyDeviceToHost, st));
+    HIPCHK(hipStreamSynchronize(st));
+    counts2[0] = (int64_t)h_cnt[0]; counts2[1] = (int64_t)h_cnt[1];
+    return MTTS_OK;
+}
+
+int32_t mtts_debug_w_seal_stats(MttsEngine* e, int64_t* out10) {
+    if (!e || !out10) return fail(MTTS_EINVAL, "null argument");
+    if (!e->w_seal_done) return fail(MTTS_ESTATE, "the weights are not sealed (mtts_weights_ready has not run since the last bind)");
+    for (int i = 0; i < 3; ++i) {
+        out10[2 * i] = (int64_t)e->w_seal_cnt[i][0];
+        out10[2 * i + 1] = (int64_t)e->w_seal_cnt[i][1];
+        out10[6 + i] = e->w_seal_on[i];
+    }
+    out10[9] = (int64_t)e->w_seal_bytes;
+    return MTTS_OK;
+}
 int32_t mtts_k_gemm_swiglu_bf16(const void* w, const void* x, void* y, int32_t M, int32_t N, int32_t K, void* stream) {
     if (!w || !x || !y || M < 1 || M > MTTS_RCAP || K % 16 || N < 32 || N % 32) return fail(MTTS_EINVAL, "gemm_swiglu: need 1<=M<=128, K%%16==0, N%%32==0");
     hipStream_t st = S(stream);
@@ -39,7 +112,9 @@
     TRY(hb.get((uint16_t**)&op, (size_t)tp * 32 * (N / 2)));
     launch_pack_weight(w, wp, N, K, N, 1, 0, st);
     launch_pack_rows(x, xp, M, K, tp, st);
-    launch_gemm(EPI_SILU, tiles, p, wp, xp, K, N, N, nullptr, (uint16_t*)op, st);
+    void* ws = nullptr;
+    TRY(hook_w_seal(hb, EPI_SILU, tiles, p, wp, K, N, N, st, &ws));
+    launch_gemm(EPI_SILU, tiles, p, wp, xp, K, N, N, nullptr, (uint16_t*)op, st, ws);
     launch_unpack_rows(op, y, M, N / 2, st);
     HIPCHK(hipGetLastError());
     HIPCHK(hipStreamSynchronize(st));
@@ -424,11 +499,14 @@
     HIPCHK(hipMemset(x, 0x3c, (size_t)MTTS_PFCAP * K * 2));
     TRY(hb.get(&out, (size_t)MTTS_PFCAP * N));
     TRY(hb.get(&part, (size_t)p.ksplit * MTTS_PFCAP * N));
+    std::vector<void*> ws(copies, nullptr);
+    if (!tile_rows)
+        for (int i = 0; i < copies; ++i) TRY(hook_w_seal(hb, epi, 1, p, w[i], K, N, N, nullptr, &ws[i]));
     hipEvent_t e0, e1;
     hipEventCreate(&e0); hipEventCreate(&e1);
     auto go = [&](int i) {
         if (tile_rows) launch_gemm_tile(epi, tile_rows, p.ksplit, w[i % copies], x, K, N, N, part, out, nullptr);
-        else launch_gemm(epi, 1, p, w[i % copies], x, K, N, N, part, out, nullptr);
+        else launch_gemm(epi, 1, p, w[i % copies], x, K, N, N, part, out, nullptr, ws[i % copies]);
     };
     for (int i = 0; i < copies; ++i) go(i);
     HIPCHK(hipDeviceSynchronize());
diff --git a/moss-ttsd_amd/csrc/launch.h b/moss-ttsd_amd/csrc/launch.h
--- a/moss-ttsd_amd/csrc/launch.h
+++ b/moss-ttsd_amd/csrc/launch.h
@@ -13,7 +13,11 @@
 GemmPlan mtts_plan_gemm(int Npad, int K, int want_ksplit);
 GemmPlan mtts_plan_gemm_forced(int Npad, int K, int ksplit, int waves);
 void launch_gemm(int epi, int mb, const GemmPlan& p, const void* Wp, const void* Xp, int K, int Npad, int n_valid,
-                 float* partial, uint16_t* out, hipStream_t st);
+                 float* partial, uint16_t* out, hipStream_t st, const void* Ws = nullptr);
+int mtts_w_seal_depth(int epi, const GemmPlan& p, int K, int Npad, int n_valid);
+size_t mtts_w_seal_bytes(int Npad, int K, int T);
+void launch_w_seal(const void* Wp, void* Ws, int Npad, int K, int T, unsigned long long* cnt, hipStream_t st);
+long long mtts_w_seal_launches();
 int mtts_tile_ksplit(int Npad, int K, int R);
 void launch_gemm_tile(int epi, int R, int ksplit, const void* Wp, const void* Xp, int K, int Npad, int n_valid,
                       float* partial, uint16_t* out, hipStream_t st);
diff --git a/moss-ttsd_amd/csrc/seal.h b/moss-ttsd_amd/csrc/seal.h
--- /dev/null
+++ b/moss-ttsd_amd/csrc/seal.h
@@ -0,0 +1,79 @@
+#pragma once
+#include "common.h"
+
+__device__ __forceinline__ uint32_t u4c(const u32x4_t& v, int c) { return c == 0 ? v.x : c == 1 ? v.y : c == 2 ? v.z : v.w; }
+__device__ __forceinline__ void pk_unit(const u32x4_t* pk, int j, uint32_t w[4]) {
+    const uint32_t L0 = u4c(pk[j >> 1], 2 * (j & 1)), L1 = u4c(pk[j >> 1], 2 * (j & 1) + 1);
+    const uint32_t N = u4c(pk[8 + (j >> 2)], j & 3);
+    const uint32_t lo = pk[12].x, hi = pk[12].y;
+    const uint32_t HA = ((N & 0x08080808u) << 4) | __builtin_amdgcn_perm(hi, lo, N & 0x07070707u);
+    const uint32_t HB = (N & 0x80808080u) | __builtin_amdgcn_perm(hi, lo, (N >> 4) & 0x07070707u);
+    w[0] = __builtin_amdgcn_perm(HA, L0, 0x05010400u);
+    w[1] = __builtin_amdgcn_perm(HA, L0, 0x07030602u);
+    w[2] = __builtin_amdgcn_perm(HB, L1, 0x05010400u);
+    w[3] = __builtin_amdgcn_perm(HB, L1, 0x07030602u);
+}
+
+__host__ __device__ constexpr int pk_order(int i) { return i == 0 ? 12 : (i - 1) % 3 == 0 ? 8 + (i - 1) / 3 : 2 * ((i - 1) / 3) + (i - 1) % 3 - 1; }
+__device__ bool seal_encode(const u32x4_t (&v)[16], u32x4_t* __restrict__ pk, uint32_t spare, bool unfit) {
+    unsigned long long b0 = 0ull, b1 = 0ull;
+#pragma unroll
+    for (int j = 0; j < 16; ++j)
+#pragma unroll
+        for (int c = 0; c < 4; ++c)
+#pragma unroll
+            for (int h = 0; h < 2; ++h) {
+                const uint32_t e = (u4c(v[j], c) >> (8 + 16 * h)) & 0x7fu;
+                if (e & 64u) b1 |= 1ull << (e & 63u);
+                else b0 |= 1ull << e;
+            }
+    const int n0 = __popcll(b0), n = n0 + __popcll(b1);
+    if (n > 8 || unfit) {
+        pk[12 * 64] = u32x4_t{0u, 0u, spare, 1u};
+        return false;
+    }
+    unsigned long long dict = 0ull;
+    {
+        unsigned long long t0 = b0, t1 = b1;
+        for (int i = 0; i < n; ++i) {
+            uint32_t e;
+            if (t0) { e = __ffsll((long long)t0) - 1; t0 &= t0 - 1; }
+            else { e = 64 + __ffsll((long long)t1) - 1; t1 &= t1 - 1; }
+            dict |= (unsigned long long)e << (8 * i);
+        }
+    }
+    auto code = [&](uint32_t half) -> uint32_t {
+        const uint32_t e = (half >> 8) & 0x7fu;
+        const uint32_t rank = (e & 64u) ? n0 + __popcll(b1 & ((1ull << (e & 63u)) - 1ull)) : __popcll(b0 & ((1ull << e) - 1ull));
+        return ((half >> 12) & 8u) | rank;
+    };
+    uint32_t lowp[32], nib[16];
+#pragma unroll
+    for (int j = 0; j < 16; ++j) {
+        uint32_t N = 0u;
+#pragma unroll
+        for (int g = 0; g < 2; ++g) {
+            uint32_t L = 0u;
+#pragma unroll
+            for (int k = 0; k < 4; ++k) {
+                const uint32_t half = (u4c(v[j], 2 * g + (k >> 1)) >> (16 * (k & 1))) & 0xffffu;
+                L |= (half & 0xffu) << (8 * k);
+                N |= code(half) << (8 * k + 4 * g);
+            }
+            lowp[2 * j + g] = L;
+        }
+        nib[j] = N;
+    }
+#pragma unroll
+    for (int u = 0; u < 8; ++u) pk[u * 64] = u32x4_t{lowp[4 * u], lowp[4 * u + 1], lowp[4 * u + 2], lowp[4 * u + 3]};
+#pragma unroll
+    for (int u = 0; u < 4; ++u) pk[(8 + u) * 64] = u32x4_t{nib[4 * u], nib[4 * u + 1], nib[4 * u + 2], nib[4 * u + 3]};
+    pk[12 * 64] = u32x4_t{(uint32_t)dict, (uint32_t)(dict >> 32), spare, 0u};
+    return true;
+}
+__device__ bool seal_lane(const u32x4_t* __restrict__ raw, u32x4_t* __restrict__ pk) {
+    u32x4_t v[16];
+#pragma unroll
+    for (int j = 0; j < 16; ++j) v[j] = raw[j * 64];
+    return seal_encode(v, pk, 0u, false);
+}
diff --git a/moss-ttsd_amd/mtts/capi.py b/moss-ttsd_amd/mtts/capi.py
--- a/moss-ttsd_amd/mtts/capi.py
+++ b/moss-ttsd_amd/mtts/capi.py
@@ -91,6 +91,10 @@
     "mtts_k_gemm_bf16": (C.c_int32, [C.c_void_p, C.c_void_p, C.c_void_p, C.c_int32, C.c_int32, C.c_int32,
                                      C.c_int32, C.c_void_p]),
     "mtts_debug_gemm_depth_launches": (C.c_int64, []),
+    "mtts_debug_w_seal_launches": (C.c_int64, []),
+    "mtts_debug_w_seal_stats": (C.c_int32, [C.c_void_p, C.c_void_p]),
+    "mtts_k_gemm_head_bf16": (C.c_int32, [C.c_void_p, C.c_void_p, C.c_void_p, C.c_int32, C.c_int32, C.c_int32, C.c_int32, C.c_void_p]),
+    "mtts_k_w_seal": (C.c_int32, [C.c_void_p, C.c_int32, C.c_int32, C.c_int32, C.c_void_p, C.c_void_p, C.c_void_p, C.c_void_p]),
     "mtts_debug_attn_row_launches": (C.c_int64, []),
     "mtts_k_attn_section": (C.c_int32, [C.c_void_p, C.c_int32] + [C.c_void_p] * 4 + [C.c_float] + [C.c_void_p] * 4 +
                             [C.c_int32] * 6 + [C.c_void_p] * 6),
diff --git a/moss-ttsd_amd/mtts/engine.py b/moss-ttsd_amd/mtts/engine.py
--- a/moss-ttsd_amd/mtts/engine.py
+++ b/moss-ttsd_amd/mtts/engine.py
@@ -268,6 +268,13 @@
         capi.check(self.lib.mtts_debug_kv_pack_stats(self._h, o.ctypes.data))
         return dict(zip(("k_pages", "k_unsealed", "v_pages", "v_unsealed", "k_layers_on", "v_layers_on"), (int(x) for x in o)))
 
+    def w_seal_stats(self):
+        o = np.zeros(10, dtype=np.int64)
+        capi.check(self.lib.mtts_debug_w_seal_stats(self._h, o.ctypes.data))
+        d = {n: (int(o[2 * i]), int(o[2 * i + 1]), bool(o[6 + i])) for i, n in enumerate(("down", "head0", "heads17"))}
+        d["bytes"] = int(o[9])
+        return d
+
     def debug_set_kv_len(self, n):
         capi.check(self.lib.mtts_debug_set_kv_len(self._h, int(n)))
 
```

Result: no change. 82100 codec_tokens/s (median of 6 runs) (+0.3%).
